# ArturKKK/graphcast-lite

Measured on AMD Instinct MI355X. Metric: training samples/sec (6h windows) + achieved HBM GB/s on mesh GCNConv, higher is better.
Workload: dtype f32

## Files before the change

### graphcast-lite_amd/csrc/linear.hip

```cpp
#include "common.h"
#include "mfma_io.h"
#include "x3.h"

namespace {

using namespace gcl::mfma_io;

#include "gemm_tile.h"

#define gcl_lin_sync() ((abl & 8) != 0)

constexpr int lin_min_waves(int NS, int KT) { return (NS <= 2 && KT <= 64) ? 3 : (NS <= 2 && KT <= 128) ? 2 : 1; }
constexpr bool lin_zpre(int NS, int EPI) { return EPI == 1 && NS >= 4; }

template <int NS, int EPI, int KT, bool VEC>
__global__ __launch_bounds__(256, lin_min_waves(NS, KT)) void linear_mfma_kernel(const float* __restrict__ X, int64_t ldx,
                                                          const float* __restrict__ in_slope,
                                                          const float* __restrict__ W, int32_t ldw, int32_t trans,
                                                          const float* __restrict__ bias, float* __restrict__ Y,
                                                          int64_t ldy, int64_t rows, int32_t K, int32_t N,
                                                          const float* __restrict__ Z, int64_t ldz,
                                                          const float* __restrict__ z_slope,
                                                          double* __restrict__ slope_part, int32_t akind,
                                                          int32_t abl) {
// ... 1032 lines not shown
  g->KT = K <= 64 ? 64 : K <= 128 ? 128 : 256;
  const int KP = ((K + 3) & ~3) + 2;
  g->waves = 4;
  g->lds = ((size_t)g->NS * 32 + 128) * KP * sizeof(float) + 64;
  if (g->lds > gcl::kLdsBytes) {
    g->waves = 2;
    g->lds = ((size_t)g->NS * 32 + 64) * KP * sizeof(float) + 64;
  }
  GCL_CHECK_ARG(g->lds <= gcl::kLdsBytes, "linear: K=%d N=%d needs %zu B of LDS (>160 KiB)", K, N, g->lds);
  int bpc = (int)(gcl::kLdsBytes / g->lds);
  const int by_regs = lin_min_waves(g->NS, g->KT) * 4 / g->waves;
  if (bpc > by_regs) bpc = by_regs;
  if (bpc < 1) bpc = 1;
  const int64_t ntiles = gcl::cdiv(rows, 32 * g->waves);
  const int64_t cap = (int64_t)gcl::kNumCU * bpc;
  g->grid = (int)(ntiles < cap ? ntiles : cap);
  return GCL_OK;
}

template <int EPI>
int launch_linear(const float* X, int64_t ldx, const float* in_slope, const float* W, int ldw, int trans,
                  const float* bias, float* Y, int64_t ldy, int64_t rows, int K, int N, const float* Z, int64_t ldz,
                  const float* z_slope, double* slope_part, int* nparts, hipStream_t st, int akind) {
  if (rows == 0) {
    if (nparts) *nparts = 0;
    return GCL_OK;
  }
  if (use_valu()) {
    const int64_t total = rows * N;
    int grid = (int)(gcl::cdiv(total, 256) < 4096 ? gcl::cdiv(total, 256) : 4096);
    hipLaunchKernelGGL((linear_valu_kernel<EPI>), dim3(grid), dim3(256), 0, st, X, ldx, in_slope, W, ldw, trans,
                       bias, Y, ldy, rows, K, N, Z, ldz, z_slope, slope_part, akind);
    GCL_CHECK_LAUNCH();
    if (nparts) *nparts = grid;
    return GCL_OK;
  }
  const int vec_x = (K % 4 == 0) && (ldx % 4 == 0) && gcl::aligned16(X);
  LinGeom g;
  int rc = lin_geom(rows, K, N, vec_x != 0, &g);
  if (rc) return rc;
#define GCL_LIN3(NS_, KT_, V_)                                                                                    \
  do {                                                                                                            \
    auto kern = linear_mfma_kernel<NS_, EPI, KT_, V_>;                                                            \
    GCL_ENSURE_DYN_LDS(kern, gcl::kLdsBytes);                                                                     \
    hipLaunchKernelGGL(kern, dim3(g.grid), dim3(g.waves * 64), g.lds, st, X, ldx, in_slope, W, ldw, trans, bias,  \
                       Y, ldy, rows, K, N, Z, ldz, z_slope, slope_part, akind, gcl_ablate());                     \
  } while (0)
#define GCL_LIN2(NS_, KT_)                 \
  do {                                     \
    if (vec_x) GCL_LIN3(NS_, KT_, true);   \
    else GCL_LIN3(NS_, KT_, false);        \
  } while (0)
#define GCL_LIN(NS_)                                \
  do {                                              \
    if (g.KT == 64) GCL_LIN2(NS_, 64);              \
    else if (g.KT == 128) GCL_LIN2(NS_, 128);       \
    else GCL_LIN3(NS_, 256, true);                  \
  } while (0)
  switch (g.NS) {
    case 1: GCL_LIN(1); break;
    case 2: GCL_LIN(2); break;
    case 4: GCL_LIN(4); break;
    default: GCL_LIN(8); break;
  }
#undef GCL_LIN3
#undef GCL_LIN
#undef GCL_LIN2
  GCL_CHECK_LAUNCH();
  if (nparts) *nparts = g.grid;
  return GCL_OK;
}

bool panel_fits(int K, int N, bool vec_x, bool trans, bool w_ok) {
  const int impl = gcl::env_is("GCL_DENSE_IMPL", "tile") ? 1 : gcl::env_is("GCL_DENSE_IMPL", "panel") ? 2 : 0;
  const bool tile_ok = vec_x && w_ok && K % 4 == 0 && N % 4 == 0;
  if (impl == 1 && tile_ok) return false;
  if (impl == 0 && tile_ok && (K > 128 || (N >= 128 && (K >= 128 || trans)))) return false;
  if (K < 1 || K > 256 || N < 1 || N > 256) return false;
  if (!vec_x && K > 128) return false;
  int NS = (N + 31) / 32;
  if (NS == 3) NS = 4;
  if (NS > 4) NS = 8;
  const int KP = ((K + 3) & ~3) + 2;
  return ((size_t)NS * 32 + 64) * KP * sizeof(float) + 64 <= gcl::kLdsBytes;
}

template <int EPI>
int launch_gemm(const float* X, int64_t ldx, int akind, const float* slope, const float* W, int64_t ldw, int trans,
                const float* bias, float* Y, int64_t ldy, int64_t rows, int K, int N, const float* Z, int64_t ldz,
                const float* add, int64_t ldadd, double* slope_part, int* nparts, hipStream_t st) {
  if (nparts) *nparts = 0;
  if (rows == 0) return GCL_OK;
  GCL_CHECK_ARG((K % 4 == 0) && (ldx % 4 == 0) && gcl::aligned16(X), "dense: wide shapes need K %% 4 == 0 and 16-B aligned rows (K=%d ldx=%lld)", K, (long long)ldx);
  GCL_CHECK_ARG((ldw % 4 == 0) && gcl::aligned16(W) && (!trans || N % 4 == 0), "dense: wide shapes need a 16-B aligned weight block (ldw=%lld N=%d)", (long long)ldw, N);
  GtGeom g = gt_geom(rows, N);
  const int x3_tile = gcl::env_int("GCL_X3", 1) != 0 && gcl::env_int("GCL_X3_TILE", 1) != 0;
  if (x3_tile && !trans && g.mi == 2) {
    auto kern = gemm_tile_x3_kernel<EPI>;
    GCL_ENSURE_DYN_LDS(kern, gcl::kLdsBytes);
    hipLaunchKernelGGL(kern, dim3(g.grid), dim3(256), gtx3_lds(), st, X, ldx, akind, slope, W, ldw, bias, Y, ldy, rows, K, N,
                       Z, ldz, add, ldadd, slope_part, g.nt, g.total, g.per_xcd);
    GCL_CHECK_LAUNCH();
    if (nparts) *nparts = (int)g.grid;
    return GCL_OK;
  }
#define GCL_GT(T_, MI_)                                                                                           \
  do {                                                                                                            \
    auto kern = gemm_tile_kernel<EPI, T_, MI_>;                                                                   \
    GCL_ENSURE_DYN_LDS(kern, gcl::kLdsBytes);                                                                     \
    hipLaunchKernelGGL(kern, dim3(g.grid), dim3(256), gt_lds(MI_), st, X, ldx, akind, slope, W, ldw, bias, Y, ldy, \
                       rows, K, N, Z, ldz, add, ldadd, slope_part, g.nt, g.total, g.per_xcd);                     \
  } while (0)
  if (trans) {
    if (g.mi == 1) GCL_GT(true, 1);
    else GCL_GT(true, 2);
  } else {
    if (g.mi == 1) GCL_GT(false, 1);
    else GCL_GT(false, 2);
  }
#undef GCL_GT
  GCL_CHECK_LAUNCH();
  if (nparts) *nparts = (int)g.grid;
  return GCL_OK;
}

}

extern "C" size_t gcl_colsum_ws_bytes(int64_t, int32_t);
extern "C" int gcl_colsum(const float*, int64_t, int64_t, int32_t, float*, int32_t, void*, size_t, gcl_stream_t);

static int check_act(const char* who, int act, const float* slope) {
  GCL_CHECK_ARG(act == GCL_ACT_NONE || act == GCL_ACT_PRELU || act == GCL_ACT_SILU, "%s: unknown activation %d", who, act);
  GCL_CHECK_ARG(act != GCL_ACT_PRELU || slope, "%s: GCL_ACT_PRELU needs the slope pointer", who);
  return GCL_OK;
}

extern "C" int gcl_dense_fwd(const float* x, int64_t ldx, int32_t act, const float* slope, const float* W, int64_t ldw,
                             const float* bias, const float* addend, int64_t ldadd, float* y, int64_t ldy,
                             int64_t rows, int32_t Fin, int32_t Fout, gcl_stream_t stream) {
  GCL_CHECK_ARG(x && W && y, "dense_fwd: null argument");
  GCL_CHECK_ARG(rows >= 0 && Fin >= 1 && Fout >= 1 && ldx >= Fin && ldy >= Fout && ldw >= Fin && (!addend || ldadd >= Fout),
                "dense_fwd: bad shape rows=%lld ldx=%lld ldy=%lld ldw=%lld", (long long)rows, (long long)ldx,
                (long long)ldy, (long long)ldw);
  if (int rc = check_act("dense_fwd", act, slope)) return rc;
  const bool vec_x = (Fin % 4 == 0) && (ldx % 4 == 0) && gcl::aligned16(x);
  if (!addend && ldw == Fin && !use_valu() && gcl::x3_linear_fwd_applicable(x, ldx, y, ldy, Fin, Fout, act))
    return gcl::x3_linear_fwd(x, ldx, act, act == GCL_ACT_PRELU ? slope : nullptr, W, bias, y, ldy, rows, Fin, Fout,
                              (hipStream_t)stream);
  if (!addend && ldw == Fin && (use_valu() || panel_fits(Fin, Fout, vec_x, false, (ldw % 4 == 0) && gcl::aligned16(W))))
    return launch_linear<EPI_BIAS>(x, ldx, act == GCL_ACT_PRELU ? slope : nullptr, W, Fin, 0, bias, y, ldy, rows, Fin,
                                   Fout, nullptr, 0, nullptr, nullptr, nullptr, (hipStream_t)stream, act);
  return launch_gemm<EPI_BIAS>(x, ldx, act, act == GCL_ACT_PRELU ? slope : nullptr, W, ldw, 0, bias, y, ldy, rows, Fin,
                               Fout, nullptr, 0, addend, ldadd, nullptr, nullptr, (hipStream_t)stream);
}

extern "C" int gcl_linear_fwd(const float* x, int64_t ldx, const float* in_slope, const float* W, const float* bias,
                              float* y, int64_t ldy, int64_t rows, int32_t Fin, int32_t Fout, gcl_stream_t stream) {
  return gcl_dense_fwd(x, ldx, in_slope ? GCL_ACT_PRELU : GCL_ACT_NONE, in_slope, W, Fin, bias, nullptr, 0, y, ldy, rows,
                       Fin, Fout, stream);
}

static size_t slope_parts_cap(int64_t rows, int32_t Fin) {
  const int64_t g = (int64_t)gt_geom(rows, Fin).grid;
  return (size_t)(g > 4096 ? g : 4096);
}

extern "C" size_t gcl_linear_bwd_ws_bytes(int64_t rows, int32_t Fin, int32_t Fout) {
  size_t nc = (size_t)(Fin + 31) / 32;
  if (nc > 4) nc = 4;
  const size_t FinP = nc * 32;
  size_t no = (size_t)(Fout + 31) / 32;
  no = no <= 2 ? no : no <= 4 ? 4 : 8;
  const size_t FoutP = no * 32;
  const size_t dw = (size_t)kDwBlocks * FoutP * (FinP + 1) * sizeof(float);
  const size_t sl = slope_parts_cap(rows, Fin) * sizeof(double);
  return dw + sl;
}

extern "C" int gcl_dense_bwd_dx(const float* dy, int64_t lddy, const float* W, int64_t ldw, const float* z, int64_t ldz,
                                int32_t act, const float* slope, float* d_slope, const float* addend, int64_t ldadd,
                                float* dx, int64_t lddx, int64_t rows, int32_t Fin, int32_t Fout, void* ws,
                                size_t ws_bytes, gcl_stream_t stream) {
  GCL_CHECK_ARG(dy && W && dx, "dense_bwd_dx: null argument");
  GCL_CHECK_ARG(lddy >= Fout && lddx >= Fin && ldw >= Fin && (!addend || ldadd >= Fin), "dense_bwd_dx: leading dimension too small");
  if (int rc = check_act("dense_bwd_dx", act, slope)) return rc;
  GCL_CHECK_ARG(act == GCL_ACT_NONE || (z && ldz >= Fin), "dense_bwd_dx: activation given without its pre-activation z");
  hipStream_t st = (hipStream_t)stream;
  const float* sl = act == GCL_ACT_PRELU ? slope : nullptr;
  double* slope_part = nullptr;
  if (sl && d_slope) {
    GCL_CHECK_ARG(ws && ws_bytes >= slope_parts_cap(rows, Fin) * sizeof(double) && gcl::aligned16(ws), "dense_bwd_dx: workspace too small");
    slope_part = (double*)ws;
  }
  int nparts = 0, rc;
  const float* zz = act == GCL_ACT_NONE ? nullptr : z;
  const bool vec_x = (Fout % 4 == 0) && (lddy % 4 == 0) && gcl::aligned16(dy);
  if (!addend && ldw == Fin && (use_valu() || panel_fits(Fout, Fin, vec_x, true, (ldw % 4 == 0) && gcl::aligned16(W))))
    rc = launch_linear<EPI_DX>(dy, lddy, nullptr, W, Fin, 1, nullptr, dx, lddx, rows, Fout, Fin, zz, ldz, sl, slope_part,
                               &nparts, st, act);
  else {
    const size_t off = (slope_parts_cap(rows, Fin) * sizeof(double) + 255) & ~(size_t)255;
    const size_t need = off + (size_t)Fin * Fout * sizeof(float);
    if (ws && ws_bytes >= need && gcl::aligned16(ws) && Fout % 4 == 0 && rows >= 4096) {
      float* Wt = reinterpret_cast<float*>(static_cast<char*>(ws) + off);
      hipLaunchKernelGGL(transpose_kernel, dim3((unsigned)gcl::cdiv(Fin, 32), (unsigned)gcl::cdiv(Fout, 32)), dim3(256), 0,
                         st, W, ldw, Wt, Fout, Fin);
      rc = launch_gemm<EPI_DX>(dy, lddy, act, sl, Wt, Fout, 0, nullptr, dx, lddx, rows, Fout, Fin, zz, ldz, addend,
                               ldadd, slope_part, &nparts, st);
    } else {
      rc = launch_gemm<EPI_DX>(dy, lddy, act, sl, W, ldw, 1, nullptr, dx, lddx, rows, Fout, Fin, zz, ldz, addend, ldadd,
                               slope_part, &nparts, st);
    }
  }
  if (rc) return rc;
  if (slope_part && nparts > 0) {
    hipLaunchKernelGGL(reduce_scalar_kernel, dim3(1), dim3(64), 0, st, slope_part, nparts, d_slope);
    GCL_CHECK_LAUNCH();
  }
  return GCL_OK;
}

extern "C" int gcl_linear_bwd_dx(const float* dy, int64_t lddy, const float* W, const float* x, int64_t ldx,
                                 const float* in_slope, float* d_in_slope, float* dx, int64_t lddx, int64_t rows,
                                 int32_t Fin, int32_t Fout, void* ws, size_t ws_bytes, gcl_stream_t stream) {
  GCL_CHECK_ARG(!in_slope || (x && ldx >= Fin), "linear_bwd_dx: in_slope given without the forward input x");
  return gcl_dense_bwd_dx(dy, lddy, W, Fin, in_slope ? x : nullptr, ldx, in_slope ? GCL_ACT_PRELU : GCL_ACT_NONE,
                          in_slope, d_in_slope, nullptr, 0, dx, lddx, rows, Fin, Fout, ws, ws_bytes, stream);
}

static int dw_block(const float* dy, int64_t lddy, const float* x, int64_t ldx, int akind, const float* in_slope,
                    float* dW, int64_t lddw, float* db, int64_t rows, int32_t Fin, int32_t Fout, int32_t accumulate,
                    void* ws, hipStream_t st) {
  const int nct = (Fin + 127) / 128;
  const int NC = nct > 1 ? 4 : (Fin + 31) / 32;
  int NO = (Fout + 31) / 32;
  NO = NO <= 2 ? NO : NO <= 4 ? 4 : 8;
  const int FinP = NC * 32, FoutP = NO * 32;
  const size_t lds = (size_t)kDwRT * (FoutP + FinP) * sizeof(float);
  const int64_t cap = (lds > 80 * 1024 ? gcl::kNumCU : kDwBlocks) / nct;
  int64_t nblk = gcl::cdiv(rows, (nct > 1 ? 4 : 2) * kDwRT);
  if (nblk > cap) nblk = cap;
  if (nblk < 1) nblk = 1;
  int64_t rpb = gcl::cdiv(rows, nblk);
  rpb = gcl::cdiv(rpb, kDwRT) * kDwRT;
  nblk = rows > 0 ? gcl::cdiv(rows, rpb) : 1;
  float* part = (float*)ws;
  float* dbpart = part + (size_t)kDwBlocks * FoutP * FinP;
  const int64_t tile_stride = (int64_t)nblk * FoutP * FinP;
  const bool vec = (lddy % 4 == 0) && (ldx % 4 == 0) && gcl::aligned16(dy) && gcl::aligned16(x);
#define GCL_DW3(NO_, NC_, V_)                                                                                     \
  do {                                                                                                            \
    auto kern = dw_mfma_kernel<NO_, NC_, V_>;                                                                     \
    GCL_ENSURE_DYN_LDS(kern, gcl::kLdsBytes);                                                                     \
    hipLaunchKernelGGL(kern, dim3((unsigned)nblk, (unsigned)nct), dim3(256), lds, st, dy, lddy, x, ldx, in_slope, part, \
                       db ? dbpart : nullptr, rows, Fin, Fout, rpb, akind, tile_stride);                          \
  } while (0)
#define GCL_DW2(NO_, NC_)              \
  do {                                 \
    if (vec) GCL_DW3(NO_, NC_, true);  \
    else GCL_DW3(NO_, NC_, false);     \
  } while (0)
#define GCL_DW(NO_)                    \
  do {                                 \
    switch (NC) {                      \
      case 1: GCL_DW2(NO_, 1); break;  \
      case 2: GCL_DW2(NO_, 2); break;  \
      case 3: GCL_DW2(NO_, 3); break;  \
      default: GCL_DW2(NO_, 4); break; \
    }                                  \
  } while (0)
  switch (NO) {
    case 1: GCL_DW(1); break;
    case 2: GCL_DW(2); break;
    case 4: GCL_DW(4); break;
    default: GCL_DW(8); break;
  }
#undef GCL_DW
#undef GCL_DW2
#undef GCL_DW3
  GCL_CHECK_LAUNCH();
  for (int ct = 0; ct < nct; ct += 3) {
    RedSeg seg[3] = {{nullptr, 0, 0, 1, 0, 0, 0}, {nullptr, 0, 0, 1, 0, 0, 0}, {nullptr, 0, 0, 1, 0, 0, 0}};
    for (int q = 0; q < 3 && ct + q < nct; ++q) {
      const int c = ct + q;
      const int fi = Fin - c * 128 < 128 ? Fin - c * 128 : 128;
      GCL_CHECK_ARG((int64_t)c * tile_stride < ((int64_t)1 << 31), "dense_bwd_dw: partial workspace offset overflows");
      seg[q] = RedSeg{dW + c * 128, (int32_t)(c * tile_stride), Fout * FinP, FinP, fi, (int32_t)lddw, accumulate};
    }
    launch_reduce_multi(part, (int)nblk, (int64_t)FoutP * FinP, seg[0], seg[1], seg[2], st);
    GCL_CHECK_LAUNCH();
  }
  if (db) return gcl::launch_reduce_parts(dbpart, (int)nblk, (int64_t)FoutP, FoutP, db, Fout, 1, Fout, accumulate, st);
  return GCL_OK;
}

extern "C" int gcl_dense_bwd_dw(const float* dy, int64_t lddy, const float* x, int64_t ldx, int32_t act,
                                const float* slope, float* dW, int64_t lddw, float* db, int64_t rows, int32_t Fin,
                                int32_t Fout, int32_t accumulate, void* ws, size_t ws_bytes, gcl_stream_t stream) {
  GCL_CHECK_ARG(dy && x && dW, "dense_bwd_dw: null argument");
  GCL_CHECK_ARG(lddy >= Fout && ldx >= Fin && lddw >= Fin, "dense_bwd_dw: leading dimension too small");
  GCL_CHECK_ARG(Fin >= 1 && Fout >= 1, "dense_bwd_dw: bad shape");
  GCL_CHECK_ARG(lddw < (1 << 30), "dense_bwd_dw: lddw too large");
  if (int rc = check_act("dense_bwd_dw", act, slope)) return rc;
  GCL_CHECK_ARG(ws && ws_bytes >= gcl_linear_bwd_ws_bytes(rows, Fin, Fout), "dense_bwd_dw: workspace too small");
  const float* sl = act == GCL_ACT_PRELU ? slope : nullptr;
  for (int o0 = 0; o0 < Fout; o0 += 256) {
    const int fo = Fout - o0 < 256 ? Fout - o0 : 256;
    int rc = dw_block(dy + o0, lddy, x, ldx, act, sl, dW + (int64_t)o0 * lddw, lddw, db ? db + o0 : nullptr, rows, Fin,
                      fo, accumulate, ws, (hipStream_t)stream);
    if (rc) return rc;
  }
  return GCL_OK;
}

extern "C" int gcl_linear_bwd_dw(const float* dy, int64_t lddy, const float* x, int64_t ldx, const float* in_slope,
                                 float* dW, float* db, int64_t rows, int32_t Fin, int32_t Fout, int32_t accumulate,
                                 void* ws, size_t ws_bytes, gcl_stream_t stream) {
  return gcl_dense_bwd_dw(dy, lddy, x, ldx, in_slope ? GCL_ACT_PRELU : GCL_ACT_NONE, in_slope, dW, Fin, db, rows, Fin,
                          Fout, accumulate, ws, ws_bytes, stream);
}

static bool fused_ok(const float* dy, int64_t lddy, const float* x, int64_t ldx, const float* dx, int64_t lddx,
                     int32_t Fin, int32_t Fout) {
  const int off = gcl::env_int("GCL_NO_FUSED_BWD", 0) != 0;
  if (off || use_valu()) return false;
  return Fout <= 64 && Fin <= 96 && (lddy >= ((Fout + 3) & ~3)) && (Fin % 4 == 0) && (lddy % 4 == 0) && (ldx % 4 == 0) &&
         (lddx >= Fin) && gcl::aligned16(dy) && gcl::aligned16(x) && dx != nullptr;
}

extern "C" size_t gcl_linear_bwd_all_ws_bytes(int64_t rows, int32_t Fin, int32_t Fout) {
  const size_t FiP = (size_t)((Fin + 31) / 32) * 32, FoP = (size_t)((Fout + 31) / 32) * 32;
  const size_t fused = (size_t)3 * gcl::kNumCU * (FoP * FiP + FoP + FiP) * sizeof(float) + (size_t)3 * gcl::kNumCU * 8 + 64;
  size_t sep = gcl_linear_bwd_ws_bytes(rows, Fin, Fout);
  const size_t cs = gcl_colsum_ws_bytes(rows, Fin);
  if (cs > sep) sep = cs;
  return fused > sep ? fused : sep;
}

static int bwd_all_impl(const float* dy, int64_t lddy, const float* W, const float* x, int64_t ldx,
                        const float* in_slope, float* d_in_slope, float* dx, int64_t lddx, float* dW,
                        float* db, float* colsum_dx, int64_t rows, int32_t Fin, int32_t Fout,
                        int32_t accumulate, void* ws, size_t ws_bytes, gcl_stream_t stream, gcl_reduce_job* job) {
  if (job) memset(job, 0, sizeof(*job));
  GCL_CHECK_ARG(dy && W && x && dx && dW, "linear_bwd_all: null argument");
  GCL_CHECK_ARG(ws && ws_bytes >= gcl_linear_bwd_all_ws_bytes(rows, Fin, Fout), "linear_bwd_all: workspace too small");
  hipStream_t st = (hipStream_t)stream;
  const int acc_dw = (accumulate & GCL_ACC_DW) ? 1 : 0, acc_db = (accumulate & GCL_ACC_DB) ? 1 : 0,
            acc_cs = (accumulate & GCL_ACC_COLSUM) ? 1 : 0;
  if (!fused_ok(dy, lddy, x, ldx, dx, lddx, Fin, Fout) || rows == 0) {
    int rc;
    if (db && acc_db != acc_dw) {
      rc = gcl_linear_bwd_dw(dy, lddy, x, ldx, in_slope, dW, nullptr, rows, Fin, Fout, acc_dw, ws, ws_bytes, stream);
      if (rc) return rc;
      rc = gcl_colsum(dy, lddy, rows, Fout, db, acc_db, ws, ws_bytes, stream);
    } else {
      rc = gcl_linear_bwd_dw(dy, lddy, x, ldx, in_slope, dW, db, rows, Fin, Fout, acc_dw, ws, ws_bytes, stream);
    }
    if (rc) return rc;
    rc = gcl_linear_bwd_dx(dy, lddy, W, in_slope ? x : nullptr, ldx, in_slope, d_in_slope, dx, lddx, rows, Fin, Fout,
                           ws, ws_bytes, stream);
    if (rc) return rc;
    if (colsum_dx) rc = gcl_colsum(dx, lddx, rows, Fin, colsum_dx, acc_cs, ws, ws_bytes, stream);
    return rc;
  }
  const int NO = (Fout + 31) / 32, NC = (Fin + 31) / 32;
  const int FoP = NO * 32, FiP = NC * 32;
  const int no64 = gcl::env_int("GCL_NO_FUSED64", 0) != 0;
  const bool use64 = (NC == 2) && !no64;
  const bool use_x3 = use64 && gcl::x3_linear_bwd_applicable(dy, lddy, x, ldx, dx, lddx, Fin, Fout);
  const int64_t ntiles = gcl::cdiv(rows, use64 ? 64 : 128);
  const int64_t cap = use64 ? 3 * gcl::kNumCU : gcl::kNumCU;
  const int nblk = use_x3 ? gcl::x3_linear_bwd_blocks(rows) : (int)(ntiles < cap ? ntiles : cap);
  const size_t rec_f = (size_t)FoP * FiP + FoP + FiP;
  float* part_dw = (float*)ws;
  float* part_db = part_dw + (size_t)FoP * FiP;
  float* part_cs = part_db + FoP;
  double* part_sl = (double*)(((uintptr_t)(part_dw + (size_t)3 * gcl::kNumCU * rec_f) + 15) & ~(uintptr_t)15);
  const bool want_slope = in_slope && d_in_slope;
  if (use_x3) {
    if (int rc = gcl::x3_linear_bwd(dy, lddy, W, x, ldx, in_slope, dx, lddx, rows, Fin, Fout, part_dw, db ? part_db : nullptr,
                                    colsum_dx ? part_cs : nullptr, want_slope ? part_sl : nullptr, st))
      return rc;
  } else if (use64) {
    const size_t lds64 = ((size_t)FiP * (FoP + 2) + 64 * (size_t)(FoP + 2) + 64 * (size_t)FiP) * sizeof(float);
#define GCL_FB64(NO_)                                                                                             \
  do {                                                                                                            \
    auto kern = linear_bwd_fused64_kernel<NO_>;                                                                   \
    hipLaunchKernelGGL(kern, dim3(nblk), dim3(256), lds64, st, dy, lddy, W, x, ldx, in_slope, dx, lddx, rows, Fin, \
                       Fout, part_dw, db ? part_db : nullptr, colsum_dx ? part_cs : nullptr,                      \
                       want_slope ? part_sl : nullptr);                                                           \
  } while (0)
    if (NO == 1) GCL_FB64(1);
    else GCL_FB64(2);
#undef GCL_FB64
  } else {
  const size_t lds = ((size_t)FiP * (FoP + 2) + 128 * (size_t)(FoP + 2) + 128 * (size_t)FiP) * sizeof(float);
#define GCL_FB(NO_, NC_)                                                                                          \
  do {                                                                                                            \
    auto kern = linear_bwd_fused_kernel<NO_, NC_>;                                                                \
    GCL_ENSURE_DYN_LDS(kern, gcl::kLdsBytes);                                                                     \
    hipLaunchKernelGGL(kern, dim3(nblk), dim3(256), lds, st, dy, lddy, W, x, ldx, in_slope, dx, lddx, rows, Fin,  \
                       Fout, part_dw, db ? part_db : nullptr, colsum_dx ? part_cs : nullptr,                      \
                       want_slope ? part_sl : nullptr);                                                           \
  } while (0)
  if (NO == 1 && NC == 1) GCL_FB(1, 1);
  else if (NO == 1 && NC == 2) GCL_FB(1, 2);
  else if (NO == 1 && NC == 3) GCL_FB(1, 3);
  else if (NO == 2 && NC == 1) GCL_FB(2, 1);
  else if (NO == 2 && NC == 2) GCL_FB(2, 2);
  else GCL_FB(2, 3);
#undef GCL_FB
  }
  GCL_CHECK_LAUNCH();
  {
    const int64_t rec = (int64_t)FoP * FiP + FoP + FiP;
    RedSeg s0{dW, 0, Fout * FiP, FiP, Fin, Fin, acc_dw};
    RedSeg s1{db, FoP * FiP, db ? Fout : 0, FoP, Fout, 0, acc_db};
    RedSeg s2{colsum_dx, FoP * FiP + FoP, colsum_dx ? Fin : 0, FiP, Fin, 0, acc_cs};
    if (job) {
      s1.count = db ? FoP : 0;
      s2.count = colsum_dx ? FiP : 0;
      job->part = part_dw;
      job->nparts = nblk;
      job->pstride = rec;
      const RedSeg* ss[3] = {&s0, &s1, &s2};
      for (int q = 0; q < 3; ++q) {
        job->seg[q].out = ss[q]->out;
        job->seg[q].poff = ss[q]->poff;
        job->seg[q].count = ss[q]->count;
        job->seg[q].pld = ss[q]->pld;
        job->seg[q].cols = ss[q]->cols;
        job->seg[q].ldo = ss[q]->ldo;
        job->seg[q].acc = ss[q]->acc;
      }
      job->spart = want_slope ? part_sl : nullptr;
      job->ns = want_slope ? nblk : 0;
      job->sout = want_slope ? d_in_slope : nullptr;
      return GCL_OK;
    }
    launch_reduce_multi(part_dw, nblk, rec, s0, s1, s2, st, want_slope ? part_sl : nullptr, nblk, d_in_slope);
    GCL_CHECK_LAUNCH();
  }
  return GCL_OK;
}

extern "C" int gcl_linear_bwd_all(const float* dy, int64_t lddy, const float* W, const float* x, int64_t ldx,
                                  const float* in_slope, float* d_in_slope, float* dx, int64_t lddx, float* dW,
                                  float* db, float* colsum_dx, int64_t rows, int32_t Fin, int32_t Fout,
                                  int32_t accumulate, void* ws, size_t ws_bytes, gcl_stream_t stream) {
  return bwd_all_impl(dy, lddy, W, x, ldx, in_slope, d_in_slope, dx, lddx, dW, db, colsum_dx, rows, Fin, Fout,
                      accumulate, ws, ws_bytes, stream, nullptr);
}

extern "C" int gcl_linear_bwd_all_deferred(const float* dy, int64_t lddy, const float* W, const float* x, int64_t ldx,
                                           const float* in_slope, float* d_in_slope, float* dx, int64_t lddx,
                                           float* dW, float* db, float* colsum_dx, int64_t rows, int32_t Fin,
                                           int32_t Fout, int32_t accumulate, void* ws, size_t ws_bytes,
                                           gcl_stream_t stream, gcl_reduce_job* job) {
  GCL_CHECK_ARG(job, "linear_bwd_all_deferred: null job");
  return bwd_all_impl(dy, lddy, W, x, ldx, in_slope, d_in_slope, dx, lddx, dW, db, colsum_dx, rows, Fin, Fout,
                      accumulate, ws, ws_bytes, stream, job);
}

extern "C" int gcl_reduce_jobs(const gcl_reduce_job* jobs, int32_t n, gcl_stream_t stream) {
  GCL_CHECK_ARG(n >= 0 && (jobs || n == 0), "reduce_jobs: null argument");
  hipStream_t st = (hipStream_t)stream;
  for (int32_t q = 0; q < n;) {
    RedJobsK J;
    memset(&J, 0, sizeof(J));
    int nb = 0, cnt = 0;
    bool any_slope = false;
    for (; q < n && cnt < kJobsPerLaunch; ++q) {
      const gcl_reduce_job& g = jobs[q];
      if (g.nparts <= 0) continue;
      GCL_CHECK_ARG(g.part && g.pstride % 4 == 0 && gcl::aligned16(g.part), "reduce_jobs: bad partial buffer");
      RedJobK& k = J.j[cnt];
      k.part = g.part;
      k.pstride = g.pstride;
      RedSeg* ss[3] = {&k.s0, &k.s1, &k.s2};
      int total = 0;
      for (int t = 0; t < 3; ++t) {
        GCL_CHECK_ARG((g.seg[t].poff | g.seg[t].count) % 4 == 0, "reduce_jobs: segment not 16-byte granular");
        *ss[t] = RedSeg{g.seg[t].out, g.seg[t].poff, g.seg[t].out ? g.seg[t].count : 0, g.seg[t].pld > 0 ? g.seg[t].pld : 1,
                        g.seg[t].cols, g.seg[t].ldo, g.seg[t].acc};
        total += ss[t]->count;
      }
      k.spart = g.spart;
      k.sout = g.sout;
      k.nparts = g.nparts;
      k.ns = g.ns;
      k.blk0 = nb;
      any_slope = any_slope || (g.spart && g.sout && g.ns > 0);
      if (!(g.spart && g.sout && g.ns > 0)) k.spart = nullptr;
      nb += (int)gcl::cdiv(total, 32);
      ++cnt;
    }
    if (cnt == 0) continue;
    J.n = cnt;
    J.nblk = nb;
    hipLaunchKernelGGL(reduce_jobs_kernel, dim3((unsigned)nb + (any_slope ? 1u : 0u)), dim3(256), 0, st, J);
    GCL_CHECK_LAUNCH();
  }
  return GCL_OK;
}
```

### graphcast-lite_amd/csrc/linear_x3.hip

```cpp
#include "mfma_io.h"
#include "x3.h"

namespace {

typedef unsigned int u32x2 __attribute__((ext_vector_type(2)));

#ifndef GCL_X3_ST_AUX
#define GCL_X3_ST_AUX 2
#endif
__device__ __forceinline__ float4 ld_stream(const float4* p) {
#ifndef GCL_X3_LD_PLAIN
  typedef float lv4f __attribute__((ext_vector_type(4)));
  const lv4f v = __builtin_nontemporal_load(reinterpret_cast<const lv4f*>(p));
  return make_float4(v.x, v.y, v.z, v.w);
#else
  return *p;
#endif
}
using namespace gcl::mfma_io;
using namespace gcl::x3;

constexpr int kRowB = 144;
constexpr int kImgB = 32 * kRowB;
constexpr int kTileB = 3 * kImgB;

__device__ unsigned long long x3_stamps[8 * 4096];
#ifdef GCL_STAMPS
#define X3_STAMP(slot)                                                           \
  do {                                                                           \
    __builtin_amdgcn_sched_barrier(0);                                           \
    unsigned long long t_;                                                       \
    asm volatile("s_memtime %0\n\ts_waitcnt lgkmcnt(0)" : "=s"(t_)::"memory"); \
    __builtin_amdgcn_sched_barrier(0);                                           \
    stamp_acc[slot] += t_ - stamp_last;                                          \
    stamp_last = t_;                                                             \
  } while (0)
#else
#define X3_STAMP(slot) do {} while (0)
#endif

template <int NS, bool SILU, int NKS>
__global__ __launch_bounds__(256, 2) void linear_x3_fwd_kernel(const float* __restrict__ X, int64_t ldx,
                                                               const float* __restrict__ slope_p, int32_t akind,
                                                               const float* __restrict__ W,
                                                               const float* __restrict__ bias, float* __restrict__ Y,
                                                               int64_t ldy, int64_t rows, int32_t K, int32_t N,
                                                               int32_t abl) {
  extern __shared__ __align__(16) unsigned char smem8[];
#ifdef GCL_STAMPS
  const unsigned long long stamp_t0 = __builtin_amdgcn_s_memtime();
#endif
  const int tid = threadIdx.x, lane = tid & 63, wave = __builtin_amdgcn_readfirstlane(tid >> 6);
  unsigned char* Aw = smem8 + wave * kTileB;
  const int fo = (lane & 31) * kRowB + (lane >> 5) * 16;
  const bool no_mfma = (abl & 2) != 0;
  const int64_t rows_ld = (abl & 4) ? 0 : rows;

  bf16x8 wf[NS][NKS][3];
  {
    constexpr int kWimgB = NS * 32 * kRowB;
    float2 wv[NS * 4];
#pragma unroll
    for (int i = 0; i < NS * 4; ++i) {
      const int idx = i * 256 + tid;
      const int j = idx >> 5, k = (idx & 31) * 2;
      const bool okj = j < N;
      wv[i].x = (okj && k < K) ? W[(int64_t)j * K + k] : 0.f;
      wv[i].y = (okj && k + 1 < K) ? W[(int64_t)j * K + k + 1] : 0.f;
    }
#pragma unroll
    for (int i = 0; i < NS * 4; ++i) {
      const int idx = i * 256 + tid;
      const int j = idx >> 5, k = (idx & 31) * 2;
      const Pk3 p = split2(wv[i].x, wv[i].y);
      unsigned char* d = smem8 + j * kRowB + k * 2;
      *reinterpret_cast<unsigned*>(d) = p.h;
      *reinterpret_cast<unsigned*>(d + kWimgB) = p.m;
      *reinterpret_cast<unsigned*>(d + 2 * kWimgB) = p.l;
    }
    __syncthreads();
#pragma unroll
    for (int t = 0; t < NS; ++t)
#pragma unroll
      for (int s = 0; s < NKS; ++s)
#pragma unroll
        for (int p = 0; p < 3; ++p)
          wf[t][s][p] = *reinterpret_cast<const bf16x8*>(smem8 + p * kWimgB + t * 32 * kRowB + fo + s * 32);
    __syncthreads();
  }

  const float pa = (akind == gcl::kActPrelu) ? *slope_p : 1.f;
  float4 bq;
  {
    const int oc = (lane % (NS * 8)) * 4;
    bq.x = (bias && oc < N) ? bias[oc] : 0.f;
    bq.y = (bias && oc + 1 < N) ? bias[oc + 1] : 0.f;
    bq.z = (bias && oc + 2 < N) ? bias[oc + 2] : 0.f;
    bq.w = (bias && oc + 3 < N) ? bias[oc + 3] : 0.f;
  }

  const int rsub = lane >> 4, csub = lane & 15;
  const bool cok = csub * 4 < K;
  float4 pre[8];
  auto issue = [&](int64_t tile) {
    const int64_t r0 = tile * 128 + wave * 32;
#pragma unroll
    for (int it = 0; it < 8; ++it) {
      const int64_t row = r0 + it * 4 + rsub;
      const float4* p = (cok && row < rows_ld) ? reinterpret_cast<const float4*>(X + row * ldx + csub * 4) : zero4;
      pre[it] = ld_stream(p);
    }
  };
  auto commit = [&]() {
#pragma unroll
    for (int it = 0; it < 8; ++it) {
      float4 v = pre[it];
      if (SILU) {
        v.x = gcl::silu_f(v.x); v.y = gcl::silu_f(v.y); v.z = gcl::silu_f(v.z); v.w = gcl::silu_f(v.w);
      } else {
        const float mx = v.x * pa, my = v.y * pa, mz = v.z * pa, mw = v.w * pa;
        v.x = v.x > 0.f ? v.x : mx; v.y = v.y > 0.f ? v.y : my;
        v.z = v.z > 0.f ? v.z : mz; v.w = v.w > 0.f ? v.w : mw;
      }
      const Pk3 p01 = split2(v.x, v.y), p23 = split2(v.z, v.w);
      unsigned char* d = Aw + (it * 4 + rsub) * kRowB + csub * 8;
      *reinterpret_cast<u32x2*>(d) = u32x2{p01.h, p23.h};
      *reinterpret_cast<u32x2*>(d + kImgB) = u32x2{p01.m, p23.m};
      *reinterpret_cast<u32x2*>(d + 2 * kImgB) = u32x2{p01.l, p23.l};
    }
  };

  const int64_t ntiles = (rows + 127) / 128;
  issue(blockIdx.x);
#ifdef GCL_STAMPS
  unsigned long long stamp_acc[8] = {0, 0, 0, 0, 0, 0, 0, 0}, stamp_last = __builtin_amdgcn_s_memtime();
  stamp_acc[6] = stamp_last - stamp_t0;
  stamp_acc[7] = stamp_t0;
#endif
  for (int64_t t = blockIdx.x; t < ntiles; t += gridDim.x) {
    __builtin_amdgcn_fence(__ATOMIC_ACQ_REL, "wavefront");
    X3_STAMP(0);
#ifdef GCL_STAMPS
    asm volatile("s_waitcnt vmcnt(0)" ::: "memory");
#endif
    X3_STAMP(1);
    commit();
    X3_STAMP(2);
    issue(t + gridDim.x);
    X3_STAMP(3);

    f32x16 acc[NS];
#pragma unroll
    for (int s = 0; s < NS; ++s)
#pragma unroll
      for (int r = 0; r < 16; ++r) acc[s][r] = 0.f;
    if (!no_mfma) {
#pragma unroll
      for (int s = 0; s < NKS; ++s) {
        const unsigned char* ap = Aw + fo + s * 32;
        const bf16x8 ah = *reinterpret_cast<const bf16x8*>(ap);
        const bf16x8 am = *reinterpret_cast<const bf16x8*>(ap + kImgB);
        const bf16x8 al = *reinterpret_cast<const bf16x8*>(ap + 2 * kImgB);
#pragma unroll
        for (int c = 0; c < NS; ++c) acc[c] = mfma_lo(acc[c], ah, am, al, wf[c][s][0], wf[c][s][1], wf[c][s][2]);
      }
#pragma unroll
      for (int s = 0; s < NKS; ++s) {
        const unsigned char* ap = Aw + fo + s * 32;
        const bf16x8 ah = *reinterpret_cast<const bf16x8*>(ap);
        const bf16x8 am = *reinterpret_cast<const bf16x8*>(ap + kImgB);
#pragma unroll
        for (int c = 0; c < NS; ++c) acc[c] = mfma_mid(acc[c], ah, am, wf[c][s][0], wf[c][s][1]);
      }
#pragma unroll
      for (int s = 0; s < NKS; ++s) {
        const bf16x8 ah = *reinterpret_cast<const bf16x8*>(Aw + fo + s * 32);
#pragma unroll
        for (int c = 0; c < NS; ++c) acc[c] = mfma_hi(acc[c], ah, wf[c][s][0]);
      }
    }

#ifdef GCL_STAMPS
    asm volatile("" ::"v"(acc[0][0]));
#endif
    X3_STAMP(4);
    const int64_t r0 = t * 128 + wave * 32;
    const int64_t nr64 = rows - r0;
    const int nr = nr64 < 0 ? 0 : (nr64 < 32 ? (int)nr64 : 32);
    constexpr int OS = NS * 32, LPO = OS / 4, RPP = 64 / LPO;
    float* Ot = reinterpret_cast<float*>(Aw);
#pragma unroll
    for (int s = 0; s < NS; ++s)
#pragma unroll
      for (int r = 0; r < 16; ++r) Ot[d_row(r, lane) * OS + s * 32 + (lane & 31)] = acc[s][r];
    const __amdgpu_buffer_rsrc_t ry = make_rsrc(Y + r0 * ldy, (nr > 0 && !(abl & 1)) ? ((int64_t)(nr - 1) * ldy + N) * 4 : 0);
    const int orow = lane / LPO, ocol = (lane % LPO) * 4;
#pragma unroll
    for (int p = 0; p < 32 / RPP; ++p) {
      const int i = p * RPP + orow;
      float4 v = *reinterpret_cast<const float4*>(Ot + i * OS + ocol);
      v.x += bq.x; v.y += bq.y; v.z += bq.z; v.w += bq.w;
      buf_st4<GCL_X3_ST_AUX>(ry, (ocol < N) ? (unsigned)((i * ldy + ocol) * 4) : kOOB, v);
    }
    X3_STAMP(5);
  }
#ifdef GCL_STAMPS
  if (lane == 0 && blockIdx.x < 1024)
    for (int i = 0; i < 8; ++i) x3_stamps[(blockIdx.x * 4 + wave) * 8 + i] = stamp_acc[i];
#endif
}

constexpr int kBRowB = 128;
constexpr int kImg64B = 64 * kBRowB;
__device__ __forceinline__ int swz(int r) { return (((r >> 1) & 1) << 2) | (((r >> 3) & 1) << 1) | ((r >> 2) & 1); }
__device__ __forceinline__ int sw_off(int r, int b) { return r * kBRowB + ((((b >> 4) ^ swz(r)) << 4) | (b & 15)); }

typedef short s16x4 __attribute__((ext_vector_type(4)));
__device__ __forceinline__ bf16x8 tr_frag(const unsigned char* base, int o0, int o1) {
  typedef __attribute__((address_space(3))) s16x4 lds_s16x4;
  const s16x4 a = __builtin_amdgcn_ds_read_tr16_b64_v4i16((lds_s16x4*)(base + o0));
  const s16x4 b = __builtin_amdgcn_ds_read_tr16_b64_v4i16((lds_s16x4*)(base + o1));
  return __builtin_shufflevector(a, b, 0, 1, 2, 3, 4, 5, 6, 7);
}

template <int NO>
__global__ __launch_bounds__(256, 2) void linear_x3_bwd_kernel(
    const float* __restrict__ dY, int64_t lddy, const float* __restrict__ W, const float* __restrict__ P,
    int64_t ldp, const float* __restrict__ in_slope, float* __restrict__ dX, int64_t lddx, int64_t rows, int32_t Fin,
    int32_t Fout, float* __restrict__ part_dw, float* __restrict__ part_db, float* __restrict__ part_cs,
    double* __restrict__ part_slope) {
  constexpr int FoP = NO * 32, FiP = 64, NKO = NO * 2, NT = NO * 2;
  extern __shared__ __align__(16) unsigned char smem8[];
  unsigned char* Yimg = smem8;
  unsigned char* Pimg = smem8 + 3 * kImg64B;
  float* Stg = reinterpret_cast<float*>(smem8 + 6 * kImg64B);
  const int tid = threadIdx.x, lane = tid & 63, wave = __builtin_amdgcn_readfirstlane(tid >> 6);
  const int li = lane & 31, h = lane >> 5;
  const int rg = wave & 1, sg = wave >> 1;
  const int so = wave % NO, sc = wave / NO;
  const bool has_tile = wave < NT;

  bf16x8 wtf[NKO][3];
  {
    float2 wv[8];
#pragma unroll
    for (int i = 0; i < 8; ++i) {
      const int idx = i * 256 + tid;
      const int c = idx & 63, o = (idx >> 6) * 2;
      wv[i].x = (c < Fin && o < Fout) ? W[(int64_t)o * Fin + c] : 0.f;
      wv[i].y = (c < Fin && o + 1 < Fout) ? W[(int64_t)(o + 1) * Fin + c] : 0.f;
    }
#pragma unroll
    for (int i = 0; i < 8; ++i) {
      const int idx = i * 256 + tid;
      const int c = idx & 63, o = (idx >> 6) * 2;
      const Pk3 p = split2(wv[i].x, wv[i].y);
      unsigned char* d = Yimg + sw_off(c, o * 2);
      *reinterpret_cast<unsigned*>(d) = p.h;
      *reinterpret_cast<unsigned*>(d + kImg64B) = p.m;
      *reinterpret_cast<unsigned*>(d + 2 * kImg64B) = p.l;
    }
    __syncthreads();
#pragma unroll
    for (int s = 0; s < NKO; ++s)
#pragma unroll
      for (int p = 0; p < 3; ++p)
        wtf[s][p] = *reinterpret_cast<const bf16x8*>(Yimg + p * kImg64B + sw_off(32 * sg + li, (16 * s + 8 * h) * 2));
    __syncthreads();
  }

  const bool act = in_slope != nullptr;
  const float slope = act ? *in_slope : 1.f;
  const int64_t ntiles = (rows + 63) / 64;

  const int rsub = lane >> 4, csub = lane & 15;
  const bool yok = csub * 4 < Fout, pok = csub * 4 < Fin;
  const unsigned ym0 = csub * 4 < Fout ? ~0u : 0u, ym1 = csub * 4 + 1 < Fout ? ~0u : 0u, ym2 = csub * 4 + 2 < Fout ? ~0u : 0u,
                 ym3 = csub * 4 + 3 < Fout ? ~0u : 0u;
  float4 pre_y[4], pre_p[4];
  auto issue = [&](int64_t tile) {
    const int64_t r0 = tile * 64 + wave * 16;
#pragma unroll
    for (int it = 0; it < 4; ++it) {
      const int64_t row = r0 + it * 4 + rsub;
      const bool rok = row < rows;
      pre_y[it] = ld_stream((yok && rok) ? reinterpret_cast<const float4*>(dY + row * lddy + csub * 4) : zero4);
      pre_p[it] = ld_stream((pok && rok) ? reinterpret_cast<const float4*>(P + row * ldp + csub * 4) : zero4);
    }
  };

  int fo[NKO];
#pragma unroll
  for (int s = 0; s < NKO; ++s) fo[s] = sw_off(rg * 32 + li, (2 * s + h) * 16);
  const int g = lane >> 4, i16 = lane & 15;
  int troY[2], troP[2];
#pragma unroll
  for (int j = 0; j < 2; ++j) {
    const int r = 8 * (g >> 1) + 4 * j + (i16 >> 2), b = 32 * (g & 1) + 8 * (i16 & 3);
    troY[j] = sw_off(r, 64 * so + b);
    troP[j] = sw_off(r, 64 * sc + b);
  }

  f32x16 dw_hi, dw_lo;
#pragma unroll
  for (int r = 0; r < 16; ++r) dw_hi[r] = 0.f, dw_lo[r] = 0.f;
  float4 db4 = make_float4(0.f, 0.f, 0.f, 0.f), cs4 = make_float4(0.f, 0.f, 0.f, 0.f);
  double slope_acc = 0.0;
  float4 cur_p[4];

  issue(blockIdx.x);
#ifdef GCL_STAMPS
  unsigned long long stamp_acc[8] = {0, 0, 0, 0, 0, 0, 0, 0}, stamp_last = __builtin_amdgcn_s_memtime();
#endif
  for (int64_t t = blockIdx.x; t < ntiles; t += gridDim.x) {
#ifdef GCL_STAMPS
    asm volatile("s_waitcnt vmcnt(0)" ::: "memory");
#endif
    X3_STAMP(0);
#pragma unroll
    for (int it = 0; it < 4; ++it) {
      float4 y = pre_y[it];
      y.x = __uint_as_float(__float_as_uint(y.x) & ym0); y.y = __uint_as_float(__float_as_uint(y.y) & ym1);
      y.z = __uint_as_float(__float_as_uint(y.z) & ym2); y.w = __uint_as_float(__float_as_uint(y.w) & ym3);
      db4.x += y.x; db4.y += y.y; db4.z += y.z; db4.w += y.w;
      const float4 z = pre_p[it];
      cur_p[it] = z;
      float4 a;
      {
        const float mx = z.x * slope, my = z.y * slope, mz = z.z * slope, mw = z.w * slope;
        a.x = z.x > 0.f ? z.x : mx; a.y = z.y > 0.f ? z.y : my; a.z = z.z > 0.f ? z.z : mz; a.w = z.w > 0.f ? z.w : mw;
      }
      const Pk3 y01 = split2(y.x, y.y), y23 = split2(y.z, y.w), a01 = split2(a.x, a.y), a23 = split2(a.z, a.w);
      const int off = sw_off(wave * 16 + it * 4 + rsub, csub * 8);
      *reinterpret_cast<u32x2*>(Yimg + off) = u32x2{y01.h, y23.h};
      *reinterpret_cast<u32x2*>(Yimg + off + kImg64B) = u32x2{y01.m, y23.m};
      *reinterpret_cast<u32x2*>(Yimg + off + 2 * kImg64B) = u32x2{y01.l, y23.l};
      *reinterpret_cast<u32x2*>(Pimg + off) = u32x2{a01.h, a23.h};
      *reinterpret_cast<u32x2*>(Pimg + off + kImg64B) = u32x2{a01.m, a23.m};
      *reinterpret_cast<u32x2*>(Pimg + off + 2 * kImg64B) = u32x2{a01.l, a23.l};
    }
    X3_STAMP(1);
    __syncthreads();
    X3_STAMP(2);
    issue(t + gridDim.x);
    X3_STAMP(3);

    {
      f32x16 acc;
#pragma unroll
      for (int r = 0; r < 16; ++r) acc[r] = 0.f;
#pragma unroll
      for (int s = 0; s < NKO; ++s) {
        const bf16x8 ah = *reinterpret_cast<const bf16x8*>(Yimg + fo[s]);
        const bf16x8 am = *reinterpret_cast<const bf16x8*>(Yimg + fo[s] + kImg64B);
        const bf16x8 al = *reinterpret_cast<const bf16x8*>(Yimg + fo[s] + 2 * kImg64B);
        acc = mfma_lo(acc, ah, am, al, wtf[s][0], wtf[s][1], wtf[s][2]);
      }
#pragma unroll
      for (int s = 0; s < NKO; ++s) {
        const bf16x8 ah = *reinterpret_cast<const bf16x8*>(Yimg + fo[s]);
        const bf16x8 am = *reinterpret_cast<const bf16x8*>(Yimg + fo[s] + kImg64B);
        acc = mfma_mid(acc, ah, am, wtf[s][0], wtf[s][1]);
      }
#pragma unroll
      for (int s = 0; s < NKO; ++s) acc = mfma_hi(acc, *reinterpret_cast<const bf16x8*>(Yimg + fo[s]), wtf[s][0]);
#pragma unroll
      for (int r = 0; r < 16; ++r) Stg[(rg * 32 + d_row(r, lane)) * 64 + sg * 32 + li] = acc[r];
    }

    X3_STAMP(4);
    if (has_tile) {
#pragma unroll
      for (int s = 0; s < 4; ++s) {
        const unsigned char* ya = Yimg + s * 16 * kBRowB;
        const unsigned char* pa = Pimg + s * 16 * kBRowB;
        const bf16x8 ah = tr_frag(ya, troY[0], troY[1]), am = tr_frag(ya + kImg64B, troY[0], troY[1]),
                     al = tr_frag(ya + 2 * kImg64B, troY[0], troY[1]);
        const bf16x8 bh = tr_frag(pa, troP[0], troP[1]), bm = tr_frag(pa + kImg64B, troP[0], troP[1]),
                     bl = tr_frag(pa + 2 * kImg64B, troP[0], troP[1]);
        dw_lo = mfma_lo(dw_lo, ah, am, al, bh, bm, bl);
        dw_lo = mfma_mid(dw_lo, ah, am, bh, bm);
        dw_hi = mfma_hi(dw_hi, ah, bh);
      }
    }
#ifdef GCL_STAMPS
    asm volatile("" ::"v"(dw_hi[0]), "v"(dw_lo[0]));
#endif
    X3_STAMP(5);
    __syncthreads();
    X3_STAMP(6);

    {
      const int64_t r0 = t * 64;
      const int64_t nr = (rows - r0) < 64 ? (rows - r0) : 64;
      const __amdgpu_buffer_rsrc_t rx = make_rsrc(dX + r0 * lddx, nr > 0 ? ((nr - 1) * lddx + Fin) * 4 : 0);
#pragma unroll
      for (int it = 0; it < 4; ++it) {
        const int row = wave * 16 + it * 4 + rsub;
        float4 v = *reinterpret_cast<const float4*>(Stg + row * 64 + csub * 4);
        const float4 z = cur_p[it];
        const bool nx = act && z.x <= 0.f, ny = act && z.y <= 0.f, nz = act && z.z <= 0.f, nw = act && z.w <= 0.f;
        slope_acc += (double)(((nx ? v.x * z.x : 0.f) + (ny ? v.y * z.y : 0.f)) + ((nz ? v.z * z.z : 0.f) + (nw ? v.w * z.w : 0.f)));
        v.x = nx ? v.x * slope : v.x; v.y = ny ? v.y * slope : v.y; v.z = nz ? v.z * slope : v.z; v.w = nw ? v.w * slope : v.w;
        cs4.x += v.x; cs4.y += v.y; cs4.z += v.z; cs4.w += v.w;
        buf_st4<GCL_X3_ST_AUX>(rx, pok ? (unsigned)((row * lddx + csub * 4) * 4) : kOOB, v);
      }
    }
    X3_STAMP(7);
  }
#ifdef GCL_STAMPS
  if (lane == 0 && blockIdx.x < 1024)
    for (int i = 0; i < 8; ++i) x3_stamps[(blockIdx.x * 4 + wave) * 8 + i] = stamp_acc[i];
#endif

  constexpr size_t REC = (size_t)FoP * FiP + FoP + FiP;
  float* out = part_dw + (size_t)blockIdx.x * REC;
  if (has_tile) {
#pragma unroll
    for (int r = 0; r < 16; ++r) out[(size_t)(so * 32 + d_row(r, lane)) * FiP + sc * 32 + li] = dw_hi[r] + dw_lo[r];
  }
  __syncthreads();
  float* red = reinterpret_cast<float*>(smem8);
  {
    float* rdb = red + (wave * 4 + rsub) * 64 + csub * 4;
    *reinterpret_cast<float4*>(rdb) = db4;
    *reinterpret_cast<float4*>(rdb + 16 * 64) = cs4;
  }
  for (int off = 32; off > 0; off >>= 1) slope_acc += __shfl_down(slope_acc, off, 64);
  double* dred = reinterpret_cast<double*>(red + 2 * 16 * 64);
  if (lane == 0) dred[wave] = slope_acc;
  __syncthreads();
  if (tid < 128) {
    const int which = tid >> 6, c = tid & 63;
    float s = 0.f;
#pragma unroll
    for (int q = 0; q < 16; ++q) s += red[(which * 16 + q) * 64 + c];
    if (which == 0) {
      if (part_db && c < FoP) part_db[(size_t)blockIdx.x * REC + c] = s;
    } else {
      if (part_cs) part_cs[(size_t)blockIdx.x * REC + c] = s;
    }
  }
  if (part_slope && tid == 0) part_slope[blockIdx.x] = (dred[0] + dred[1]) + (dred[2] + dred[3]);
}

int x3_ablate() {
#ifndef GCL_STAMPS
  return 0;
#endif
  static const int v = gcl::env_int("GCL_ABLATE", 0);
  return v;
}

}

#ifdef GCL_STAMPS
extern "C" int gcl_debug_read_stamps_x3(unsigned long long* host_out, int count) {
  GCL_CHECK_HIP(hipDeviceSynchronize());
  GCL_CHECK_HIP(hipMemcpyFromSymbol(host_out, HIP_SYMBOL(x3_stamps), sizeof(unsigned long long) * count));
  return GCL_OK;
}
#endif

namespace gcl {

bool x3_linear_fwd_applicable(const float* x, int64_t ldx, const float* y, int64_t ldy, int K, int N, int akind) {
  if (!env_int("GCL_X3", 1)) return false;
  if (K < 1 || K > 64 || N < 4 || N > 64 || (N & 3)) return false;
  if ((ldx & 3) || (ldy & 3) || !aligned16(x) || !aligned16(y)) return false;
  if (ldx * 4 * 35 >= ((int64_t)1 << 31) || ldy * 4 * 35 >= ((int64_t)1 << 31)) return false;
  return akind == kActNone || akind == kActPrelu || akind == kActSilu;
}

int x3_linear_fwd(const float* x, int64_t ldx, int akind, const float* slope, const float* W, const float* bias,
                  float* y, int64_t ldy, int64_t rows, int K, int N, hipStream_t st) {
  if (rows == 0) return GCL_OK;
  const int64_t ntiles = cdiv(rows, 128);
  const int grid = (int)(ntiles < 2 * kNumCU ? ntiles : 2 * kNumCU);
  const size_t lds = 4 * (size_t)kTileB;
#define GCL_X3F3(NS_, SILU_, NKS_)                                                                                \
  hipLaunchKernelGGL((linear_x3_fwd_kernel<NS_, SILU_, NKS_>), dim3(grid), dim3(256), lds, st, x, ldx, slope, akind, \
                     W, bias, y, ldy, rows, K, N, x3_ablate())
#define GCL_X3F(NS_, SILU_)           \
  do {                                \
    if (K <= 32) GCL_X3F3(NS_, SILU_, 2); \
    else GCL_X3F3(NS_, SILU_, 4);     \
  } while (0)
  if (akind == kActSilu) {
    if (N > 32) GCL_X3F(2, true);
    else GCL_X3F(1, true);
  } else {
    if (N > 32) GCL_X3F(2, false);
    else GCL_X3F(1, false);
  }
#undef GCL_X3F3
#undef GCL_X3F
  GCL_CHECK_LAUNCH();
  return GCL_OK;
}

bool x3_linear_bwd_applicable(const float* dy, int64_t lddy, const float* x, int64_t ldx, const float* dx, int64_t lddx,
                              int Fin, int Fout) {
  if (!env_int("GCL_X3", 1)) return false;
  if (Fin < 33 || Fin > 64 || (Fin & 3) || Fout < 1 || Fout > 64) return false;
  if (lddy < ((Fout + 3) & ~3) || (lddy & 3) || (ldx & 3) || (lddx & 3) || lddx < Fin) return false;
  if (!aligned16(dy) || !aligned16(x) || !aligned16(dx)) return false;
  return lddx * 4 * 70 < ((int64_t)1 << 31);
}

int x3_linear_bwd_blocks(int64_t rows) {
  const int64_t ntiles = cdiv(rows, 64);
  return (int)(ntiles < 2 * kNumCU ? ntiles : 2 * kNumCU);
}

int x3_linear_bwd(const float* dy, int64_t lddy, const float* W, const float* x, int64_t ldx, const float* in_slope,
                  float* dx, int64_t lddx, int64_t rows, int Fin, int Fout, float* part_dw, float* part_db,
                  float* part_cs, double* part_slope, hipStream_t st) {
  const int grid = x3_linear_bwd_blocks(rows);
  const size_t lds = 6 * (size_t)kImg64B + 64 * 64 * sizeof(float);
#define GCL_X3B(NO_)                                                                                              \
  do {                                                                                                            \
    auto kern = linear_x3_bwd_kernel<NO_>;                                                                        \
    GCL_ENSURE_DYN_LDS(kern, gcl::kLdsBytes);                                                                     \
    hipLaunchKernelGGL(kern, dim3(grid), dim3(256), lds, st, dy, lddy, W, x, ldx, in_slope, dx, lddx, rows, Fin, Fout, \
                       part_dw, part_db, part_cs, part_slope);                                                    \
  } while (0)
  if (Fout > 32) GCL_X3B(2);
  else GCL_X3B(1);
#undef GCL_X3B
  GCL_CHECK_LAUNCH();
  return GCL_OK;
}

}
```

### graphcast-lite_amd/csrc/x3.h

```cpp
#pragma once
#include "common.h"

namespace gcl {

bool x3_linear_fwd_applicable(const float* x, int64_t ldx, const float* y, int64_t ldy, int K, int N, int akind);
int x3_linear_fwd(const float* x, int64_t ldx, int akind, const float* slope, const float* W, const float* bias,
                  float* y, int64_t ldy, int64_t rows, int K, int N, hipStream_t st);

bool x3_linear_bwd_applicable(const float* dy, int64_t lddy, const float* x, int64_t ldx, const float* dx, int64_t lddx,
                              int Fin, int Fout);
int x3_linear_bwd_blocks(int64_t rows);
int x3_linear_bwd(const float* dy, int64_t lddy, const float* W, const float* x, int64_t ldx, const float* in_slope,
                  float* dx, int64_t lddx, int64_t rows, int Fin, int Fout, float* part_dw, float* part_db,
                  float* part_cs, double* part_slope, hipStream_t st);

}

#ifdef __HIPCC__
#include "mfma_io.h"

namespace gcl {
namespace x3 {

using mfma_io::f32x16;
typedef short bf16x8 __attribute__((ext_vector_type(8)));
typedef __bf16 bf16x2_t __attribute__((ext_vector_type(2)));
typedef float f32x2_t __attribute__((ext_vector_type(2)));

__device__ __forceinline__ unsigned pk_bf16(float a, float b) {
  return __builtin_bit_cast(unsigned, __builtin_convertvector(f32x2_t{a, b}, bf16x2_t));
}
struct Pk3 {
  unsigned h, m, l;
};
__device__ __forceinline__ Pk3 split2(float a, float b) {
  Pk3 p;
  p.h = pk_bf16(a, b);
  float ra = a - __uint_as_float(p.h << 16), rb = b - __uint_as_float(p.h & 0xffff0000u);
  p.m = pk_bf16(ra, rb);
  ra -= __uint_as_float(p.m << 16);
  rb -= __uint_as_float(p.m & 0xffff0000u);
  p.l = pk_bf16(ra, rb);
  return p;
}

__device__ __forceinline__ f32x16 mfma_lo(f32x16 acc, bf16x8 ah, bf16x8 am, bf16x8 al, bf16x8 bh, bf16x8 bm, bf16x8 bl) {
  acc = __builtin_amdgcn_mfma_f32_32x32x16_bf16(al, bh, acc, 0, 0, 0);
  acc = __builtin_amdgcn_mfma_f32_32x32x16_bf16(ah, bl, acc, 0, 0, 0);
  acc = __builtin_amdgcn_mfma_f32_32x32x16_bf16(am, bm, acc, 0, 0, 0);
  return acc;
}
__device__ __forceinline__ f32x16 mfma_mid(f32x16 acc, bf16x8 ah, bf16x8 am, bf16x8 bh, bf16x8 bm) {
  acc = __builtin_amdgcn_mfma_f32_32x32x16_bf16(am, bh, acc, 0, 0, 0);
  acc = __builtin_amdgcn_mfma_f32_32x32x16_bf16(ah, bm, acc, 0, 0, 0);
  return acc;
}
__device__ __forceinline__ f32x16 mfma_hi(f32x16 acc, bf16x8 ah, bf16x8 bh) {
  return __builtin_amdgcn_mfma_f32_32x32x16_bf16(ah, bh, acc, 0, 0, 0);
}

}
}
#endif
```

### graphcast-lite_amd/functional.py

```python
from typing import List, Optional

import os

import torch

from . import hip


def _grad_slot(p: Optional[torch.Tensor], needs: bool):
    if p is None or not needs:
        return None, False, True
    if p.grad is not None:
        return p.grad, True, True
    return torch.zeros_like(p), False, False


class _Grads:

    def __init__(self, params: List[Optional[torch.Tensor]], needs: List[bool]):
        self.dst, self.acc, self.ret_none = [], [], []
        for p, nd in zip(params, needs):
            d, a, r = _grad_slot(p, nd)
            self.dst.append(d)
            self.acc.append(a)
            self.ret_none.append(r)

    def out(self):
        return tuple(None if r else d for d, r in zip(self.dst, self.ret_none))


def _flat3(x: torch.Tensor):
    if x.dim() == 2:
        x = x.unsqueeze(0)
    if not x.is_contiguous():
        x = x.contiguous()
    return x


class MLPFn(torch.autograd.Function):
    @staticmethod
    def forward(ctx, x, owner, has_ln: bool, eps: float, *params):
        L = (len(params) - (2 if has_ln else 0) + 1) // 3
        shape = x.shape
        x2 = hip.rows2d(x.detach())
        zs = []
        cur, slope = x2, None
        for k in range(L):
            W, b = params[3 * k], params[3 * k + 1]
            z = hip.linear_fwd(cur, W.detach(), b.detach(), slope)
            zs.append(z)
            cur = z
            slope = params[3 * k + 2].detach() if k < L - 1 else None
        stats = None
        out = cur
        if has_ln:
            out, stats = hip.layernorm_fwd(cur, params[-2].detach(), params[-1].detach(), eps)
        ctx.owner, ctx.has_ln, ctx.L = owner, has_ln, L
        ctx.x2, ctx.zs, ctx.stats = x2, zs, stats
        ctx.params = params
        return out.view(shape[:-1] + (out.shape[-1],))

    @staticmethod
    def backward(ctx, dy):
        params, L = ctx.params, ctx.L
        needs = list(ctx.needs_input_grad[4:])
        G = _Grads(list(params), needs)
        dy2 = hip.rows2d(dy)
        zs = ctx.zs
        if ctx.has_ln:
            gi, bi = len(params) - 2, len(params) - 1
            dgam = G.dst[gi] if G.dst[gi] is not None else torch.zeros_like(params[gi])
            dbet = G.dst[bi] if G.dst[bi] is not None else torch.zeros_like(params[bi])
            dz = hip.layernorm_bwd(dy2, zs[-1], params[gi].detach(), ctx.stats, dgam, dbet, G.acc[gi] and G.acc[bi])
        else:
            dz = dy2
        dx = None
        for k in range(L - 1, -1, -1):
            W = params[3 * k].detach()
            inp = ctx.x2 if k == 0 else zs[k - 1]
            slope = None if k == 0 else params[3 * k - 1].detach()
            wi, bi = 3 * k, 3 * k + 1
            dW = G.dst[wi] if G.dst[wi] is not None else torch.zeros_like(params[wi])
            db = G.dst[bi]
            if k > 0:
                dz = hip.linear_bwd_all(dz, W, inp, slope, G.dst[3 * k - 1], dW, db, None, G.acc[wi], acc_db=G.acc[bi])
            elif ctx.needs_input_grad[0]:
                dx = hip.linear_bwd_all(dz, W, inp, None, None, dW, db, None, G.acc[wi], acc_db=G.acc[bi],
                                        act=hip.ACT_NONE)
            elif db is not None and G.acc[bi] != G.acc[wi]:
                hip.linear_bwd_dw(dz, inp, None, dW, None, G.acc[wi])
                hip.colsum(dz, db, G.acc[bi])
            else:
                hip.linear_bwd_dw(dz, inp, None, dW, db, G.acc[wi])
        if dx is not None:
            dx = dx.view(dy.shape[:-1] + (dx.shape[-1],))
        return (dx, None, None, None) + G.out()


_LN_COLSUM = os.environ.get("GCL_NO_LN_COLSUM", "0") in ("0", "")
_ROWS_OUT = os.environ.get("GCL_NO_ROWS_OUT", "0") in ("0", "")


def _lat_first_layer_bwd(lat, enc3, dz3, W, dW, acc_dw: bool, want_dx: bool, Pc=None, enc_shape=None):
    _, _, inv_a, inv_fold = lat.maps
    B, ne, D = enc_shape if enc3 is None else enc3.shape
    G, Md, r = lat.G, lat.Md, lat.r
    nc = Md + r
    Fo = dz3.shape[-1]
    dz3 = dz3 if dz3.is_contiguous() else dz3.contiguous()
    dzc = torch.empty(B, nc, Fo, dtype=torch.float32, device=dz3.device)
    if Md > 0:
        hip.gather2_rows(dz3, inv_a[G: G + Md], None, None, Md, B, out=dzc[:, :Md])
    if r > 1:
        hip.gather2_rows(dz3, inv_fold, None, None, B * r, B, sum_batch=True, out=dzc[:, Md:], deal=r)
    elif r == 1:
        tmp = hip.gather2_rows(dz3, inv_fold, None, None, B * r, B, sum_batch=True)
        hip.copy_rows(tmp.view(B, r, Fo), dzc[:, Md:])
    if Pc is None:
        Pc = hip.copy_rows(enc3[:, G:, :], torch.empty(B, nc, D, dtype=torch.float32, device=dz3.device))
    land = lat.landing
    shared = land is not None and land.buf is not None
    if not want_dx:
        hip.linear_bwd_dw(dzc.view(B * nc, Fo), Pc.view(B * nc, D), None, dW, None, acc_dw)
        dxc = None
    else:
        dxc = hip.linear_bwd_all(dzc.view(B * nc, Fo), W, Pc.view(B * nc, D), None, None, dW, None, None, acc_dw,
                                 act=hip.ACT_NONE).view(B, nc, D)
    if shared:
        if dxc is not None:
            hip.copy_rows(dxc, land.buf[:, G:])
        land.buf, land.mesh_pending, land.handed_over = None, False, False
        return None
    if dxc is None:
        return None
    out = torch.zeros(B, ne, D, dtype=torch.float32, device=dz3.device)
    hip.copy_rows(dxc, out[:, G:])
    return out


class LatSource:

    def __init__(self, tab, maps, M: int, G: int, Md: int, r: int, landing=None):
        self.tab, self.maps, self.M, self.G, self.Md, self.r, self.landing = tab, maps, M, G, Md, r, landing
        self._compact = {}

    def compact_tab(self, ne: int):
        t = self._compact.get(ne)
        if t is None:
            tab = self.tab.to(torch.int64)
            f = -tab - 1
            bq = torch.div(f, ne, rounding_mode="floor")
            flat_c = bq * (self.Md + self.r) + (f - bq * ne - self.G)
            t = torch.where(tab >= 0, tab - self.G, -flat_c - 1).to(torch.int32).contiguous()
            self._compact[ne] = t
        return t


class GCNStackFn(torch.autograd.Function):
    @staticmethod
    def forward(ctx, x, owner, graph, L: int, has_ln: bool, eps: float, out_rows: int, *params):
        squeeze = x.dim() == 2
        x3 = _flat3(x.detach())
        B, n, _ = x3.shape
        lat = getattr(owner, "_lat_src", None)
        if lat is not None:
            owner._lat_src = None
            n = lat.M
            if not x3.is_contiguous():
                x3 = x3.contiguous()
            if lat.landing is not None:
                lat.landing.mesh_pending = True
        ctx.lat = lat
        slope_p = params[2 * L]
        akind = getattr(owner, "act_kind", hip.ACT_PRELU)
        slope_t = slope_p.detach() if slope_p is not None else getattr(owner, "const_slope", None)
        ps = []
        cur = x3
        pad_last = None
        for k in range(L):
            W, b = params[2 * k].detach(), params[2 * k + 1].detach()
            Fout = W.shape[0]
            ldh = (Fout + 3) // 4 * 4
            act_k, slope_k = (akind, slope_t) if k > 0 else (hip.ACT_NONE, None)
            if k == 0 and lat is not None:
                p = hip.gcn_layer_fwd_tab(graph, x3, lat.tab, act_k, slope_k, W, b)
                if ldh != Fout:
                    p = p.contiguous()
                ps.append(p)
                cur = p
                continue
            if hip.gcn_layer_fusable(graph, cur, W.shape[1], Fout):
                last_rows = int(out_rows) if (k == L - 1 and out_rows and out_rows < n and not has_ln and _ROWS_OUT) else None
                p = hip.gcn_layer_fwd(graph, cur, act_k, slope_k, W, b, rows_out=last_rows)
                if k == L - 1 and ldh != Fout and not has_ln:
                    pad_last = (ldh, Fout, None)
                elif ldh != Fout:
                    p = p.contiguous()
                ps.append(p)
                cur = p
                continue
            if k == L - 1 and ldh != Fout and not has_ln:
                Wp = torch.nn.functional.pad(W, (0, 0, 0, ldh - Fout))
                bp = torch.nn.functional.pad(b, (0, ldh - Fout))
                h = hip.linear_fwd(cur.reshape(B * n, -1), Wp, None, slope_k, act=act_k)
                p = hip.aggregate(graph, h.view(B, n, ldh), bp)
                ps.append(p)
                cur = p[..., :Fout]
                pad_last = (ldh, Fout, Wp)
                continue
            h = hip.linear_fwd(cur.reshape(B * n, -1) if not cur.is_contiguous() else cur.view(B * n, -1), W, None, slope_k,
                               ld_out=ldh, act=act_k)
            h3 = torch.as_strided(h, (B, n, Fout), (n * ldh, ldh, 1))
            p = hip.aggregate(graph, h3, b)
            ps.append(p)
            cur = p
        ctx.akind, ctx.slope_t, ctx.pad_last = akind, slope_t, pad_last
        out, stats = cur, None
        ctx.land = getattr(owner, "_grad_src", None)
        if ctx.land is not None:
            owner._grad_src = None
            if has_ln and not (out_rows and out_rows < n) and not squeeze:
                ctx.land.proc_ready = True
            else:
                ctx.land = None
        if has_ln:
            land = ctx.land
            if land is not None and land.dec_buf is not None and cur.is_contiguous() and land.dec_buf.shape[2] == cur.shape[2]:
                stats = hip.layernorm_fwd_map(cur.view(B * n, -1), params[-2].detach(), params[-1].detach(), eps,
                                              land.dec_buf, land.dec_map)
                land.dec_filled = True
                out = cur.new_zeros(()).expand(B, n, cur.shape[2])
            else:
                o2, stats = hip.layernorm_fwd(cur.view(B * n, -1), params[-2].detach(), params[-1].detach(), eps)
                out = o2.view(B, n, -1)
        ctx.owner, ctx.graph, ctx.L, ctx.has_ln = owner, graph, L, has_ln
        ctx.x3, ctx.ps, ctx.stats, ctx.params, ctx.squeeze = x3, ps, stats, params, squeeze
        ctx.n_rows, ctx.out_rows = n, (int(out_rows) if out_rows and out_rows < n else 0)
        if ctx.out_rows:
            out = out[:, :ctx.out_rows, :]
        return out[0] if squeeze else out

    @staticmethod
    def backward(ctx, dy):
        params, L, graph = ctx.params, ctx.L, ctx.graph
        needs = list(ctx.needs_input_grad[7:])
        G = _Grads(list(params), needs)
        land = ctx.land
        dy_map = None
        if land is not None and land.proc_src is not None:
            if all(st == 0 for st in dy.stride()):
                dy_map = (land.proc_src, land.proc_map)
                dy3 = dy
            else:
                src, pmap = land.proc_src, land.proc_map
                dy3 = _flat3(dy) + hip.gather2_rows(src, pmap, None, None, dy.shape[-2], src.shape[0])
            land.proc_src = land.proc_map = None
            land.proc_ready = False
        else:
            dy3 = _flat3(dy)
        B, n = dy3.shape[0], ctx.n_rows
        ps = ctx.ps
        pad = ctx.pad_last
        dy_rows = dy3
        if ctx.out_rows and (ctx.has_ln or pad is None):
            dy3 = hip.pad_rows(dy3, n, dy3.shape[2])
        bi_last = 2 * L - 1
        cs_done = False
        if ctx.has_ln:
            gi, bi = len(params) - 2, len(params) - 1
            dgam = G.dst[gi] if G.dst[gi] is not None else torch.zeros_like(params[gi])
            dbet = G.dst[bi] if G.dst[bi] is not None else torch.zeros_like(params[bi])
            cs = G.dst[bi_last] if (pad is None and _LN_COLSUM) else None
            dp = hip.layernorm_bwd(None if dy_map is not None else dy3.view(B * n, -1), ps[-1].view(B * n, -1),
                                   params[gi].detach(), ctx.stats, dgam, dbet, G.acc[gi] and G.acc[bi], colsum_dx=cs,
                                   acc_colsum=bool(cs is not None and G.acc[bi_last]), dy_map=dy_map).view(B, n, -1)
            cs_done = cs is not None
        else:
            dp = dy3
        si = 2 * L
        dsl = G.dst[si] if params[si] is not None else None
        slope_t, akind = ctx.slope_t, ctx.akind
        dx = None
        Fo = params[2 * (L - 1)].shape[0]
        Fp = Fo
        if pad is not None:
            Fp = pad[0]
            dp = hip.pad_rows(dy_rows if not ctx.has_ln else dp, n, Fp)
        if G.dst[bi_last] is not None and not cs_done:
            src = dy_rows if not ctx.has_ln else dp[..., :Fo]
            hip.colsum(src.reshape(-1, Fo), G.dst[bi_last], G.acc[bi_last])
        for k in range(L - 1, -1, -1):
            W = params[2 * k].detach()
            wi = 2 * k
            inp = (ctx.x3 if k == 0 else ps[k - 1]).view(-1, (ctx.x3 if k == 0 else ps[k - 1]).shape[-1])
            dh2 = hip.aggregate(graph, dp, None, transpose=True).view(B * n, -1)
            if k == L - 1 and Fp != Fo:
# ... 470 lines not shown
```

### graphcast-lite_amd/hip.py

```python
import ctypes as C
import os
from typing import Optional

import torch

_HERE = os.path.dirname(os.path.abspath(__file__))
LIB_PATH = os.environ.get("GCL_LIB") or os.path.join(_HERE, "libgcl_hip.so")

GRAPH_GCN, GRAPH_GAT, GRAPH_MEAN = 0, 1, 2

_lib = None

_i32, _i64, _f32, _vp, _sz = C.c_int32, C.c_int64, C.c_float, C.c_void_p, C.c_size_t

_SIGNATURES = {
    "gcl_version": (C.c_int, []),
    "gcl_last_error": (C.c_char_p, []),
    "gcl_graph_count_edges": (C.c_int, [_vp, _i64, _i32, _i32, C.POINTER(_i64)]),
    "gcl_graph_build_host": (C.c_int, [_vp, _i64, _i32, _i32] + [_vp] * 8),
    "gcl_graph_create": (C.c_int, [_vp, _i64, _i32, _i32, C.POINTER(_vp)]),
    "gcl_graph_destroy": (None, [_vp]),
    "gcl_graph_num_nodes": (_i32, [_vp]),
    "gcl_graph_num_edges": (_i64, [_vp]),
    "gcl_graph_max_in_degree": (_i32, [_vp]),
    "gcl_graph_export_edges": (C.c_int, [_vp, _vp]),
    "gcl_graph_eperm_device": (_vp, [_vp]),
    "gcl_graph_halo_info": (C.c_int, [_vp, _i32, _i32, _vp]),
    "gcl_linear_fwd": (C.c_int, [_vp, _i64, _vp, _vp, _vp, _vp, _i64, _i64, _i32, _i32, _vp]),
    "gcl_linear_bwd_dx": (C.c_int, [_vp, _i64, _vp, _vp, _i64, _vp, _vp, _vp, _i64, _i64, _i32, _i32, _vp, _sz, _vp]),
    "gcl_linear_bwd_dw": (C.c_int, [_vp, _i64, _vp, _i64, _vp, _vp, _vp, _i64, _i32, _i32, _i32, _vp, _sz, _vp]),
    "gcl_linear_bwd_ws_bytes": (_sz, [_i64, _i32, _i32]),
    "gcl_linear_bwd_all": (C.c_int, [_vp, _i64, _vp, _vp, _i64, _vp, _vp, _vp, _i64, _vp, _vp, _vp, _i64, _i32, _i32,
                                     _i32, _vp, _sz, _vp]),
    "gcl_linear_bwd_all_deferred": (C.c_int, [_vp, _i64, _vp, _vp, _i64, _vp, _vp, _vp, _i64, _vp, _vp, _vp, _i64, _i32,
                                              _i32, _i32, _vp, _sz, _vp, _vp]),
    "gcl_reduce_jobs": (C.c_int, [_vp, _i32, _vp]),
    "gcl_linear_bwd_all_ws_bytes": (_sz, [_i64, _i32, _i32]),
    "gcl_aggregate": (C.c_int, [_vp, _i32, _vp, _i64, _i64, _vp, _vp, _i64, _i64, _i32, _i32, _vp]),
    "gcl_gat_fwd": (C.c_int, [_vp, _vp, _i64, _i64, _vp, _vp, _vp, _vp, _vp, _vp, _vp, _i64, _i64, _i32, _i32, _i32, _vp]),
    "gcl_gat_bwd": (C.c_int, [_vp, _vp, _i64, _i64, _vp, _i64, _i64, _vp, _vp, _vp, _vp, _vp, _vp, _i64, _i64,
                              _vp, _vp, _vp, _i32, _i32, _i32, _i32, _vp, _sz, _vp]),
    "gcl_gat_bwd_ws_bytes": (_sz, [_i64, _i32, _i32, _i32, _i32]),
    "gcl_gat_fwd_tab": (C.c_int, [_vp, _vp, _i64, _i64, _vp, _vp, _vp, _vp, _vp, _vp, _vp, _vp, _i64, _i64, _i32, _i32, _i32, _vp]),
    "gcl_gat_bwd_tab": (C.c_int, [_vp, _vp, _i64, _i64, _vp, _i64, _i64, _vp, _vp, _vp, _vp, _vp, _vp, _vp, _i64, _i64,
                                  _vp, _vp, _vp, _i32, _i32, _i32, _i32, _vp, _sz, _vp]),
    "gcl_gat_tab_ok": (C.c_int, [_vp, _i64, _i32, _i32]),
    "gcl_gat_alpha_to_edge_order": (C.c_int, [_vp, _vp, _vp, _i32, _vp]),
    "gcl_gat_prune": (C.c_int, [_vp, _vp, _f32, _vp, C.POINTER(_i64), _vp, _sz, _vp]),
    "gcl_gat_prune_ws_bytes": (_sz, [_i64]),
    "gcl_layernorm_fwd": (C.c_int, [_vp, _i64, _vp, _vp, _f32, _vp, _i64, _vp, _i64, _i32, _vp]),
    "gcl_layernorm_bwd": (C.c_int, [_vp, _i64, _vp, _i64, _vp, _vp, _vp, _i64, _vp, _vp, _i32, _i64, _i32, _vp, _sz, _vp]),
    "gcl_layernorm_bwd_cs": (C.c_int, [_vp, _i64, _vp, _i64, _vp, _vp, _vp, _i64, _vp, _vp, _vp, _i32, _i64, _i32, _vp, _sz, _vp]),
    "gcl_layernorm_bwd_map": (C.c_int, [_vp, _i64, _i64, _vp, _i32, _vp, _i64, _vp, _vp, _vp, _i64, _vp, _vp, _vp, _i32, _i64,
                                        _i32, _vp, _sz, _vp]),
    "gcl_layernorm_bwd_ws_bytes": (_sz, [_i64, _i32]),
    "gcl_graphnorm_fwd": (C.c_int, [_vp, _i64, _i64, _vp, _vp, _f32, _vp, _i64, _i64, _vp, _i32, _i32, _i32, _vp, _sz, _vp]),
    "gcl_graphnorm_bwd": (C.c_int, [_vp, _i64, _i64, _vp, _i64, _i64, _vp, _vp, _f32, _vp, _i64, _i64, _vp, _vp,
                                    _i32, _i32, _i32, _i32, _vp, _sz, _vp]),
    "gcl_graphnorm_ws_bytes": (_sz, [_i32, _i32, _i32]),
    "gcl_colsum": (C.c_int, [_vp, _i64, _i64, _i32, _vp, _i32, _vp, _sz, _vp]),
    "gcl_colsum_ws_bytes": (_sz, [_i64, _i32]),
    "gcl_assemble_input": (C.c_int, [_vp, _vp, _vp, _vp, _i64, _i32, _i32, _i32, _i32, _i32, _vp]),
    "gcl_assemble_input_tail": (C.c_int, [_vp, _vp, _vp, _vp, _i32, _vp, _i64, _i32, _i32, _i32, _i32, _i32, _vp]),
    "gcl_wmse_fwd_bwd": (C.c_int, [_vp, _i64, _i64, _vp, _i64, _i64, _vp, _i64, _i64, _vp, _vp, _f32, _f32, _vp,
                                   _vp, _vp, _vp, _i32, _i32, _i32, _vp, _sz, _vp]),
    "gcl_ar_step_bwd": (C.c_int, [_vp, _vp, _vp, _vp, _i32, _i32, _vp, _vp, _i32, _i32, _i32, _i32, _vp]),
    "gcl_pad_rows": (C.c_int, [_vp, _i64, _i64, _i32, _i32, _vp, _i64, _i64, _i32, _i32, _i32, _vp]),
    "gcl_zero": (C.c_int, [_vp, _sz, _vp]),
    "gcl_wmse_ws_bytes": (_sz, [_i32, _i32, _i32]),
    "gcl_adam_step": (C.c_int, [_vp, _vp, _vp, _vp, _i64, _f32, _f32, _f32, _f32, _f32, _i32, _f32, _vp]),
    "gcl_adam_step_dev": (C.c_int, [_vp, _vp, _vp, _vp, _i64, _f32, _f32, _f32, _f32, _f32, _vp, _vp, _f32, _vp]),
    "gcl_adam_step_groups": (C.c_int, [_vp, _vp, _vp, _vp, _i64, _vp, _i32, _vp, _vp, _vp, _vp, _f32, _f32, _f32, _f32,
                                       _f32, _vp]),
    "gcl_copy_rows": (C.c_int, [_vp, _i64, _i64, _vp, _i64, _i64, _i32, _i32, _i32, _vp]),
    "gcl_dense_fwd": (C.c_int, [_vp, _i64, _i32, _vp, _vp, _i64, _vp, _vp, _i64, _vp, _i64, _i64, _i32, _i32, _vp]),
    "gcl_dense_bwd_dx": (C.c_int, [_vp, _i64, _vp, _i64, _vp, _i64, _i32, _vp, _vp, _vp, _i64, _vp, _i64, _i64, _i32, _i32,
                                   _vp, C.c_size_t, _vp]),
    "gcl_dense_bwd_dw": (C.c_int, [_vp, _i64, _vp, _i64, _i32, _vp, _vp, _i64, _vp, _i64, _i32, _i32, _i32, _vp,
                                   C.c_size_t, _vp]),
    "gcl_gcn_layer_fwd": (C.c_int, [_vp, _vp, _i64, _i64, _i32, _vp, _vp, _vp, _vp, _i64, _i64, _i32, _i32, _i32, _i32, _vp]),
    "gcl_gcn_layer_fwd_rows": (C.c_int, [_vp, _vp, _i64, _i64, _i32, _vp, _vp, _vp, _vp, _i64, _i64, _i32, _i32, _i32, _i32, _i32, _vp]),
    "gcl_layernorm_fwd_map": (C.c_int, [_vp, _i64, _vp, _vp, _f32, _vp, _i64, _i64, _vp, _i32, _vp, _i64, _i32, _vp]),
    "gcl_gcn_layer_fwd_tab": (C.c_int, [_vp, _vp, _i64, _i64, _i64, _vp, _i32, _vp, _vp, _vp, _vp, _i64, _i64, _i32, _i32, _i32, _i32, _vp]),
    "gcl_gcn_layer_fwd_tab_ok": (C.c_int, [_vp, _i64, _i64, _i64, _i32, _i32, _i32]),
    "gcl_segment_reduce": (C.c_int, [_vp, _i64, _i64, _vp, _vp, _i32, _vp, _i64, _i64, _i32, _i32, _i32, _vp]),
    "gcl_edge_combine": (C.c_int, [_vp, _vp, _vp, _i64, _i64, _vp, _vp, _vp, _i64, _i64, _vp, _vp, _i32, _i64, _i32, _vp]),
    "gcl_act_fwd": (C.c_int, [_vp, _vp, _i64, _i32, _vp, _vp]),
    "gcl_act_bwd": (C.c_int, [_vp, _vp, _vp, _i64, _i32, _vp, _vp, _vp, C.c_size_t, _vp]),
    "gcl_act_bwd_ws_bytes": (C.c_size_t, []),
    "gcl_window_pack": (C.c_int, [_vp, _i64, _i32, _i32, _i32, _vp, _vp, _vp, _i32, _i32, _i32, _vp, _vp, _i32, _vp]),
    "gcl_ar_advance": (C.c_int, [_vp, _vp, _i64, _i64, _vp, _i64, _i64, _vp, _vp, _vp, _i64, _i64, _i32, _i32, _i32, _i32,
                                 _i32, _i32, _vp]),
    "gcl_gather2_rows": (C.c_int, [_vp, _i64, _i64, _vp, _vp, _i64, _i64, _vp, _vp, _i64, _i64, _i32, _i32, _i32, _i32, _vp]),
    "gcl_roi_gather_rows": (C.c_int, [_vp, _i32, _i32] + [_vp, _i64, _i64, _i32] * 3 + [_vp, _i64, _i64, _i32, _i32, _vp]),
    "gcl_roi_compose": (C.c_int, [_vp, _i64, _i64, _vp, _i64, _i64, _vp, _vp, _i64, _i64, _i32, _i32, _i32, _vp]),
    "gcl_segment_wsum": (C.c_int, [_vp, _i64, _i64, _i32, _i32, _vp, _vp, _vp, _vp, _i64, _i64, _vp, _i64, _i64, _i32,
                                   _i32, _i32, _i32, _vp]),
    "gcl_cross_update_fwd": (C.c_int, [_vp, _i64, _i64, _vp, _i64, _i64, _vp, _vp, _vp, _f32, _vp, _vp, _vp, _i32, _i32,
                                       _i32, _vp]),
    "gcl_nudge": (C.c_int, [_vp, _i64, _i64, _vp, _i64, _i64, _vp, _f32, _f32, _i32, _vp, _i64, _i64, _i32, _i32, _i32,
                            _vp]),
    "gcl_oi_max_stations": (C.c_int, []),
    "gcl_oi_station_cov": (C.c_int, [_vp, _vp, _i32, C.c_double, C.c_double, C.c_double, _vp, _vp]),
    "gcl_oi_factor": (C.c_int, [_vp, _i32, _vp]),
    "gcl_oi_solve": (C.c_int, [_vp, _i32, _vp, _vp, _vp, _i32, _vp]),
    "gcl_oi_innovation": (C.c_int, [_vp, _i64, _i64, _vp, _i64, _i64, _vp, _vp, _vp, _i32, _i32, _i32, _vp, _vp]),
    "gcl_oi_analysis": (C.c_int, [_vp, _i64, _i64, _vp, _i64, _i64, _vp, _i32, _vp, _vp, _vp, _vp, _i32, _vp, _vp, _vp,
                                  _vp, _i32, _f32, _f32, _f32, _f32, _i32, _vp]),
    "gcl_verify_colstats_ws_bytes": (_sz, [_i32, _i32, _i32, _i32]),
    "gcl_verify_colstats": (C.c_int, [_vp, _i64, _i64, _i32, _i32] + [_vp, _i64, _i64, _vp] * 4
                            + [_vp, _i32, _i32, _vp, _vp, _sz, _vp]),
    "gcl_verify_accumulate": (C.c_int, [_vp, _vp, _i32, _vp, _vp, _vp]),
    "gcl_regrid_blend": (C.c_int, [_vp, _i32, _i64, _i64, _i32, _vp, _vp, _i32, _i32, _vp, _i64, _i64, _vp, _vp, _i64,
                                   _i64, _vp, _i64, _i64, _i32, _vp]),
    "gcl_taper_blend": (C.c_int, [_vp, _vp, _i64, _i64, _vp, _i64, _i64, _vp, _i64, _i64, _i32, _i32, _i32, _vp]),
    "gcl_mos_forest_eval": (C.c_int, [_vp, _vp, _i32, C.c_double, _vp, _i32, _vp, _vp]),
    "gcl_mos_forest_predict": (C.c_int, [_vp, _vp, _i32, C.c_double, _vp, _i32, _i64, _i64, _i64, _i32] + [_i32] * 5
                               + [_vp, _vp, _i32, _i32, _vp, _vp, _vp, _vp, _i32, _vp]),
    "gcl_mos_idw_apply": (C.c_int, [_vp, _i32, _i64, _i64, _i64, _vp, _i64, _i64, _i64, _i32, _i32, _i32, _i32, _vp,
                                    _vp, _vp, _i32, _vp, _i32, C.c_double, C.c_double, _vp, _i32, _vp]),
    "gcl_mos_table_apply": (C.c_int, [_vp, _i32, _i64, _i64, _i64, _vp, _i64, _i64, _i64, _i32, _i32, _i32, _i32, _vp,
                                      _i32, _i32, _vp]),
}


def exported_symbols():
    return sorted(_SIGNATURES)


def lib():
    global _lib
    if _lib is None:
        if not os.path.exists(LIB_PATH):
            raise RuntimeError(
                f"{LIB_PATH} is missing: build it with `python -c 'import __graft_entry__ as g; g.build()'` "
                "(or `make -C graphcast-lite_amd/csrc`). The HIP path has no CPU fallback."
            )
        L = C.CDLL(LIB_PATH)
        for name, (res, args) in _SIGNATURES.items():
            fn = getattr(L, name)
            fn.restype = res
            fn.argtypes = args
        _lib = L
    return _lib


def _check(rc: int):
    if rc != 0:
        raise RuntimeError(f"libgcl_hip error {rc}: {lib().gcl_last_error().decode()}")


def _stream() -> int:
    return torch.cuda.current_stream().cuda_stream


def _p(t: Optional[torch.Tensor]):
    if t is None:
        return None
    if not t.is_cuda:
        raise RuntimeError("libgcl_hip needs GPU tensors (there is no CPU fallback)")
    if t.dtype != torch.float32:
        raise RuntimeError(f"libgcl_hip needs float32 tensors, got {t.dtype}")
    return t.data_ptr()


_ws = {}
_ws_retired = []


def workspace(nbytes: int, device) -> torch.Tensor:
    key = torch.device(device).index if torch.device(device).index is not None else torch.cuda.current_device()
    cur = _ws.get(key)
    if cur is None or cur.numel() < nbytes:
        size = max(int(nbytes), 1 << 20, 2 * cur.numel() if cur is not None else 0)
        if cur is not None:
            _ws_retired.append(cur)
        cur = torch.empty(size, dtype=torch.uint8, device=f"cuda:{key}")
        _ws[key] = cur
    return cur


def rows2d(t: torch.Tensor) -> torch.Tensor:
    if t.dim() == 2 and t.stride(1) == 1:
        return t
    if not t.is_contiguous():
        t = t.contiguous()
    return t.view(-1, t.shape[-1])


# ... 107 lines not shown

def _probe_begin(kind, **info):
    return PROBE.begin(kind, **info) if PROBE is not None else None


def _probe_end(tok):
    if tok is not None:
        PROBE.end(tok)


def dense_fwd(x, W, bias, act=ACT_NONE, slope=None, addend=None, out=None):
    rows, Fin = x.shape
    Fout = W.shape[0]
    assert W.shape[1] == Fin and W.stride(1) == 1 and x.stride(1) == 1
    if out is None:
        out = torch.empty(rows, Fout, dtype=torch.float32, device=x.device)
    if rows == 0:
        return out
    tok = _probe_begin("dense_fwd", rows=rows, Fin=Fin, Fout=Fout)
    _check(lib().gcl_dense_fwd(_p(x), _ld(x), int(act), _p(slope), _p(W), W.stride(0), _p(bias), _p(addend),
                               _ld(addend) if addend is not None else 0, _p(out), _ld(out), rows, Fin, Fout, _stream()))
    _probe_end(tok)
    return out


def dense_bwd_dx(dy, W, z=None, act=ACT_NONE, slope=None, d_slope=None, addend=None, out=None):
    rows, Fout = dy.shape
    Fin = W.shape[1]
    assert W.shape[0] == Fout and W.stride(1) == 1
    if out is None:
        out = torch.empty(rows, Fin, dtype=torch.float32, device=dy.device)
    if rows == 0:
        return out
    nb = lib().gcl_linear_bwd_ws_bytes(rows, Fin, Fout)
    ws = workspace(nb, dy.device)
    _check(lib().gcl_dense_bwd_dx(_p(dy), _ld(dy), _p(W), W.stride(0), _p(z), _ld(z) if z is not None else 0, int(act),
                                  _p(slope), _p(d_slope), _p(addend), _ld(addend) if addend is not None else 0, _p(out),
                                  _ld(out), rows, Fin, Fout, ws.data_ptr(), ws.numel(), _stream()))
    return out


def dense_bwd_dw(dy, x, dW, db, accumulate: bool, act=ACT_NONE, slope=None):
    rows, Fout = dy.shape
    Fin = x.shape[1]
    assert tuple(dW.shape) == (Fout, Fin) and dW.stride(1) == 1
    if rows == 0:
        if not accumulate:
            dW.zero_()
            if db is not None:
                db.zero_()
        return
    nb = lib().gcl_linear_bwd_ws_bytes(rows, Fin, Fout)
    ws = workspace(nb, dy.device)
    _check(lib().gcl_dense_bwd_dw(_p(dy), _ld(dy), _p(x), _ld(x), int(act), _p(slope), _p(dW), dW.stride(0), _p(db), rows,
                                  Fin, Fout, 1 if accumulate else 0, ws.data_ptr(), ws.numel(), _stream()))


ACC_DW, ACC_DB, ACC_COLSUM = 1, 2, 4


class _RedSeg(C.Structure):
    _fields_ = [("out", C.c_void_p), ("poff", C.c_int32), ("count", C.c_int32), ("pld", C.c_int32), ("cols", C.c_int32),
                ("ldo", C.c_int32), ("acc", C.c_int32)]


class ReduceJob(C.Structure):
    _fields_ = [("part", C.c_void_p), ("pstride", C.c_int64), ("seg", _RedSeg * 3), ("spart", C.c_void_p),
                ("sout", C.c_void_p), ("nparts", C.c_int32), ("ns", C.c_int32)]


class _Deferred:

    def __init__(self):
        self.active = False
        self.jobs, self.dests, self.pool, self.used = [], set(), [], 0
        self.keep = []

    def ws(self, nbytes, device):
        if self.used == len(self.pool):
            self.pool.append(None)
        cur = self.pool[self.used]
        if cur is None or cur.numel() < nbytes or cur.device != torch.device(device):
            if cur is not None:
                _ws_retired.append(cur)
            cur = torch.empty(int(nbytes), dtype=torch.uint8, device=device)
            self.pool[self.used] = cur
        self.used += 1
        return cur


_deferred = _Deferred()


def defer_begin():
    _deferred.active = True


def defer_flush(close: bool = True, drop: bool = False):
    d = _deferred
    try:
        if d.jobs and not drop:
            arr = (ReduceJob * len(d.jobs))(*d.jobs)
            _check(lib().gcl_reduce_jobs(C.cast(arr, C.c_void_p), len(d.jobs), _stream()))
    finally:
        d.jobs, d.dests, d.used, d.keep = [], set(), 0, []
        if close:
            d.active = False


def linear_bwd_all(dy, W, x, in_slope, d_in_slope, dW, db, colsum_dx, acc_dW: bool, acc_db=None, acc_colsum=None,
                   act=None):
    acc_db = acc_dW if acc_db is None else acc_db
    acc_colsum = acc_dW if acc_colsum is None else acc_colsum
    a = _act_of(act, in_slope)
    if a == ACT_SILU:
        if db is not None and bool(acc_db) != bool(acc_dW):
            dense_bwd_dw(dy, x, dW, None, acc_dW, a, None)
            colsum(dy, db, acc_db)
        else:
            dense_bwd_dw(dy, x, dW, db, acc_dW, a, None)
        dx = dense_bwd_dx(dy, W, x, a, None, None)
        if colsum_dx is not None:
            colsum(dx, colsum_dx, acc_colsum)
        return dx
    rows, Fout = dy.shape
    Fin = W.shape[1]
    dx = torch.empty(rows, Fin, dtype=torch.float32, device=dy.device)
    nb = lib().gcl_linear_bwd_all_ws_bytes(rows, Fin, Fout)
    acc = (ACC_DW if acc_dW else 0) | (ACC_DB if acc_db else 0) | (ACC_COLSUM if acc_colsum else 0)
    d = _deferred
    if d.active:
        dests = {t.data_ptr() for t in (dW, db, colsum_dx) if t is not None}
        if dests & d.dests:
            defer_flush(close=False)
        ws = d.ws(nb, dy.device)
        job = ReduceJob()
        _check(lib().gcl_linear_bwd_all_deferred(
            _p(dy), _ld(dy), _p(W), _p(x), _ld(x), _p(in_slope), _p(d_in_slope), _p(dx), Fin, _p(dW), _p(db),
            _p(colsum_dx), rows, Fin, Fout, acc, ws.data_ptr(), ws.numel(), _stream(), C.byref(job)))
        if job.nparts > 0:
            d.jobs.append(job)
            d.dests |= dests
            d.keep.append((dW, db, colsum_dx, d_in_slope, ws))
        else:
            d.used -= 1
        return dx
    ws = workspace(nb, dy.device)
    _check(lib().gcl_linear_bwd_all(
        _p(dy), _ld(dy), _p(W), _p(x), _ld(x), _p(in_slope), _p(d_in_slope), _p(dx), Fin, _p(dW), _p(db),
        _p(colsum_dx), rows, Fin, Fout, acc, ws.data_ptr(), ws.numel(), _stream()))
    return dx


def aggregate(graph: Graph, h3, bias, transpose=False, out=None):
    B, n, F = h3.shape
    assert n == graph.n, f"graph has {graph.n} nodes, features have {n} rows"
    assert h3.stride(2) == 1
    if out is None:
        out = torch.empty(B, n, F, dtype=torch.float32, device=h3.device)
    tok = _probe_begin("aggregate", graph=graph, transpose=bool(transpose), B=B, F=F)
    _check(lib().gcl_aggregate(graph.handle, 1 if transpose else 0, _p(h3), h3.stride(1), h3.stride(0), _p(bias),
                               _p(out), out.stride(1), out.stride(0), B, F, _stream()))
    _probe_end(tok)
    return out


def layernorm_fwd(x, gamma, beta, eps=1e-5):
    rows, F = x.shape
    y = torch.empty(rows, F, dtype=torch.float32, device=x.device)
    stats = torch.empty(rows, 2, dtype=torch.float32, device=x.device)
    _check(lib().gcl_layernorm_fwd(_p(x), _ld(x), _p(gamma), _p(beta), float(eps), _p(y), F, _p(stats), rows, F, _stream()))
    return y, stats


def layernorm_fwd_map(x, gamma, beta, eps, out3, pos):
    rows, F = x.shape
    n_per = pos.numel()
    assert out3.stride(2) == 1 and rows % n_per == 0 and out3.shape[0] == rows // n_per
    stats = torch.empty(rows, 2, dtype=torch.float32, device=x.device)
    _check(lib().gcl_layernorm_fwd_map(_p(x), _ld(x), _p(gamma), _p(beta), float(eps), _p(out3), out3.stride(1), out3.stride(0),
                                       _pi(pos), n_per, _p(stats), rows, F, _stream()))
    return stats


def layernorm_bwd(dy, x, gamma, stats, dgamma, dbeta, accumulate: bool, colsum_dx=None, acc_colsum: bool = False,
                  dy_map=None):
    rows, F = x.shape
    dx = torch.empty(rows, F, dtype=torch.float32, device=x.device)
    nb = lib().gcl_layernorm_bwd_ws_bytes(rows, F)
    ws = workspace(nb, x.device)
    acc = (ACC_DW if accumulate else 0) | (ACC_COLSUM if acc_colsum else 0)
    if dy_map is not None:
        src3, pos = dy_map
        assert src3.stride(2) == 1 and src3.shape[2] >= F and rows % pos.numel() == 0 and src3.shape[0] == rows // pos.numel()
        _check(lib().gcl_layernorm_bwd_map(_p(src3), src3.stride(1), src3.stride(0), _pi(pos), pos.numel(), _p(x), _ld(x),
                                           _p(gamma), _p(stats), _p(dx), F, _p(dgamma), _p(dbeta), _p(colsum_dx), acc, rows, F,
                                           ws.data_ptr(), ws.numel(), _stream()))
        return dx
    _check(lib().gcl_layernorm_bwd_cs(_p(dy), _ld(dy), _p(x), _ld(x), _p(gamma), _p(stats), _p(dx), F, _p(dgamma),
                                      _p(dbeta), _p(colsum_dx), acc, rows, F, ws.data_ptr(), ws.numel(), _stream()))
    return dx


def graphnorm_fwd(x3, gamma, beta, eps=1e-5):
    B, n, F = x3.shape
    y = torch.empty(B, n, F, dtype=torch.float32, device=x3.device)
    stats = torch.empty(B, 2, dtype=torch.float32, device=x3.device)
    nb = lib().gcl_graphnorm_ws_bytes(B, n, F)
    ws = workspace(nb, x3.device)
    _check(lib().gcl_graphnorm_fwd(_p(x3), x3.stride(1), x3.stride(0), _p(gamma), _p(beta), float(eps), _p(y), F, n * F,
                                   _p(stats), B, n, F, ws.data_ptr(), ws.numel(), _stream()))
    return y, stats


def graphnorm_bwd(dy3, x3, gamma, stats, dgamma, dbeta, accumulate: bool, eps=1e-5):
    B, n, F = x3.shape
    dx = torch.empty(B, n, F, dtype=torch.float32, device=x3.device)
    nb = lib().gcl_graphnorm_ws_bytes(B, n, F)
    ws = workspace(nb, x3.device)
    _check(lib().gcl_graphnorm_bwd(_p(dy3), dy3.stride(1), dy3.stride(0), _p(x3), x3.stride(1), x3.stride(0), _p(gamma),
                                   _p(stats), float(eps), _p(dx), F, n * F, _p(dgamma), _p(dbeta),
                                   1 if accumulate else 0, B, n, F, ws.data_ptr(), ws.numel(), _stream()))
    return dx


def colsum(x, out, accumulate: bool):
    rows, F = x.shape
    nb = lib().gcl_colsum_ws_bytes(rows, F)
    ws = workspace(nb, x.device)
    _check(lib().gcl_colsum(_p(x), _ld(x), rows, F, _p(out), 1 if accumulate else 0, ws.data_ptr(), ws.numel(), _stream()))
    return out


def gat_tab_ok(graph: Graph, H: int, Cc: int) -> bool:
    return bool(lib().gcl_gat_tab_ok(graph.handle, H * Cc, int(H), int(Cc)))


def gat_fwd(graph: Graph, h3, att_src, att_dst, bias, H, Cc, need_alpha=True, tab=None):
    B, n, HC = h3.shape
    if tab is not None:
        n = graph.n
        assert h3.is_contiguous()
    dev = h3.device
    a_s = torch.empty(B, n, H, dtype=torch.float32, device=dev)
    a_d = torch.empty(B, n, H, dtype=torch.float32, device=dev)
    alpha = torch.empty(B, graph.e, H, dtype=torch.float32, device=dev) if need_alpha else None
    y = torch.empty(B, n, Cc, dtype=torch.float32, device=dev)
    tok = _probe_begin("gat_fwd", graph=graph, B=B, H=H, C=Cc, alpha=need_alpha)
    if tab is not None:
        _check(lib().gcl_gat_fwd_tab(graph.handle, _p(h3), h3.stride(1), h3.stride(0), _pi(tab), _p(att_src), _p(att_dst),
                                     _p(bias), _p(a_s), _p(a_d), _p(alpha), _p(y), Cc, n * Cc, B, H, Cc, _stream()))
    else:
        _check(lib().gcl_gat_fwd(graph.handle, _p(h3), h3.stride(1), h3.stride(0), _p(att_src), _p(att_dst), _p(bias),
                                 _p(a_s), _p(a_d), _p(alpha), _p(y), Cc, n * Cc, B, H, Cc, _stream()))
    _probe_end(tok)
    return y, a_s, a_d, alpha


def gat_bwd(graph: Graph, dy3, h3, att_src, att_dst, a_s, a_d, alpha, d_att_src, d_att_dst, d_bias, accumulate, H, Cc, tab=None):
    B, n, HC = h3.shape
    if tab is not None:
        n = graph.n
    dy3 = dy3.contiguous()
    dh = torch.empty(B, n, HC, dtype=torch.float32, device=h3.device)
    nb = lib().gcl_gat_bwd_ws_bytes(graph.e, n, B, H, Cc)
    ws = workspace(nb, h3.device)
    tok = _probe_begin("gat_bwd", graph=graph, B=B, H=H, C=Cc)
    if tab is not None:
        _check(lib().gcl_gat_bwd_tab(graph.handle, _p(dy3), Cc, n * Cc, _p(h3), h3.stride(1), h3.stride(0), _pi(tab), _p(att_src),
                                     _p(att_dst), _p(a_s), _p(a_d), _p(alpha), _p(dh), HC, n * HC, _p(d_att_src),
                                     _p(d_att_dst), _p(d_bias), 1 if accumulate else 0, B, H, Cc, ws.data_ptr(), ws.numel(),
                                     _stream()))
    else:
        _check(lib().gcl_gat_bwd(graph.handle, _p(dy3), Cc, n * Cc, _p(h3), h3.stride(1), h3.stride(0), _p(att_src),
                                 _p(att_dst), _p(a_s), _p(a_d), _p(alpha), _p(dh), HC, n * HC, _p(d_att_src), _p(d_att_dst),
                                 _p(d_bias), 1 if accumulate else 0, B, H, Cc, ws.data_ptr(), ws.numel(), _stream()))
    _probe_end(tok)
    return dh


def gat_alpha_edge_order(graph: Graph, alpha_slots_1sample, H):
    out = torch.empty(graph.e, H, dtype=torch.float32, device=alpha_slots_1sample.device)
    _check(lib().gcl_gat_alpha_to_edge_order(graph.handle, _p(alpha_slots_1sample.contiguous()), _p(out), H, _stream()))
    return out


def gat_prune(graph: Graph, alpha_edges, threshold: float) -> torch.Tensor:
    buf = torch.empty(2 * graph.e, dtype=torch.int64)
    kept = _i64(0)
    nb = lib().gcl_gat_prune_ws_bytes(graph.e)
    ws = workspace(nb, alpha_edges.device)
    _check(lib().gcl_gat_prune(graph.handle, _p(alpha_edges.contiguous()), float(threshold), buf.data_ptr(),
                               C.byref(kept), ws.data_ptr(), ws.numel(), _stream()))
    k = kept.value
    return buf[: 2 * k].view(2, k).clone()


def assemble_input(x3, grid_static, mesh_static, tail3=None):
    B, G, Cdyn = x3.shape
    M, Cs = mesh_static.shape
    x3 = x3.contiguous()
    out = torch.empty(B, G + M, Cdyn + Cs, dtype=torch.float32, device=x3.device)
    if tail3 is not None and tail3.is_contiguous() and tail3.shape[2] == Cdyn + Cs:
        _check(lib().gcl_assemble_input_tail(_p(x3), _p(grid_static), _p(mesh_static), _p(tail3), tail3.shape[1], _p(out),
                                             Cdyn + Cs, B, G, M, Cdyn, Cs, _stream()))
        return out
# ... 404 lines not shown
```

### graphcast-lite_amd/models.py

```python
import contextlib
import math
import os
import sys
from collections import OrderedDict
from typing import Optional, Tuple

import numpy as np
import torch
import torch.nn as nn

from . import hip
from .config import (
    DataConfig,
    GraphBlock,
    GraphBuildingConfig,
    GraphLayerType,
    MLPBlock,
    ModelConfig,
    PipelineConfig,
)
from .create_graphs import (create_decoding_graph, create_encoding_graph, create_processing_graph,
                            create_product_graph)
from .functional import (AssembleFn, EdgeLayout, GATLayerFn, Gather2Fn, GCNStackFn, GradLanding, GraphNormFn, InteractionNetFn,
                         LatSource, LayerNormFn, MeanAggFn, MeshLatFn, MLPFn)
# ... 495 lines not shown
            return False
        def ok(m):
            node_ln = all(ln.mode == "node" for ln in m.modules() if isinstance(ln, LayerNorm))
            return m.graph_layer.layer_type == GraphLayerType.ConvGCN and node_ln

        return ok(self.encoder) and ok(self.decoder) and getattr(self, "compact", True)

    _renumber_mesh = os.environ.get("GCL_NO_RENUMBER", "0") in ("0", "")

    def _mesh_order(self):
        if not self._renumber_mesh or self.processor.graph_layer.layer_type not in (
                GraphLayerType.ConvGCN, GraphLayerType.GATConv, GraphLayerType.SparseGATConv):
            return None
        cached = getattr(self, "_mesh_perm", None)
        if cached is None:
            M = self._num_mesh_nodes
            ei = self.processing_graph.detach().cpu()
            deg = torch.bincount(ei[1], minlength=M).numpy()
            order = torch.from_numpy(np.ascontiguousarray(tile_order(self._finest_mesh.vertices, 64, degree=deg))).to(torch.int64)
            pos = torch.empty(M, dtype=torch.int64)
            pos[order] = torch.arange(M)
            cached = self._mesh_perm = (order, pos)
        return cached

    def processor_graph(self) -> torch.Tensor:
        if self._compact_eligible() and self._mesh_order() is not None and not self.using_interaction_net:
            return self._processing_graph_tiled()
        return self.processing_graph

    def _processing_graph_tiled(self):
        g = self.processing_graph
        key = (id(g), g._version)
        c = getattr(self, "_proc_tiled", None)
        if c is None or c[0] != key:
            _, pos = self._mesh_order()
            c = self._proc_tiled = (key, pos.to(g.device)[g], g)
        return c[1]

    def _processing_graph_from_tiled(self, tiled: torch.Tensor) -> torch.Tensor:
        c = getattr(self, "_proc_tiled", None)
        if c is not None and c[1] is tiled:
            return c[2]
        order, _ = self._mesh_order()
        ref = order.to(tiled.device)[tiled]
        E = ref.shape[1]
        trail = (ref[0] == ref[1]).to(torch.int32).flip(0).cumprod(0).flip(0).bool()
        col = torch.arange(E, device=ref.device)
        key = torch.where(trail, (E - trail.sum()) + ref[0], col)
        ref = ref[:, torch.argsort(key, stable=True)]
        self._proc_tiled = ((id(ref), ref._version), tiled, ref)
        return ref

    def _compact_setup(self, device):
        G, M = self._num_grid_nodes, self._num_mesh_nodes
        enc, dec = self.encoding_graph.cpu(), self.decoding_graph.cpu()
        i32 = lambda t: t.to(torch.int32).contiguous().to(device)
        md = torch.unique(enc[1]) - G
        is_dep = torch.zeros(M, dtype=torch.bool)
        is_dep[md] = True
        mi = torch.nonzero(~is_dep).flatten()
        used = torch.unique(dec[0]) - G
        Md, Mi, U = md.numel(), mi.numel(), used.numel()
        remap_e = torch.full((G + M,), -1, dtype=torch.int64)
        remap_e[:G] = torch.arange(G)
        remap_e[G + md] = G + torch.arange(Md)
        remap_d = torch.full((G + M,), -1, dtype=torch.int64)
        remap_d[:G] = torch.arange(G)
        remap_d[G + used] = G + torch.arange(U)
        c = type("Compact", (), {})()
        c.Md, c.Mi, c.U = Md, Mi, U
        c.enc_graph = remap_e[enc].contiguous().to(device)
        c.dec_graph = remap_d[dec].contiguous().to(device)
        c.empty_graph = torch.zeros(2, 0, dtype=torch.int64, device=device)
        c.mstat_dep = self.init_mesh_features[md.to(self.init_mesh_features.device)].contiguous()
        Cdyn = self._dyn_size
        inv_stat = self.init_mesh_features[mi.to(self.init_mesh_features.device)]
        c.x_inv = torch.cat([torch.zeros(Mi, Cdyn, device=device), inv_stat.to(device)], dim=1).unsqueeze(0).contiguous()
        map_a = torch.full((M,), -1, dtype=torch.int64)
        map_a[md] = G + torch.arange(Md)
        map_b = torch.full((M,), -1, dtype=torch.int64)
        map_b[mi] = torch.arange(Mi)
        inv_a = torch.full((G + Md,), -1, dtype=torch.int64)
        inv_a[G:] = md
        perm = self._mesh_order()
        c.perm = perm
        if perm is not None:
            order, pos = perm
            map_a, map_b = map_a[order], map_b[order]
            inv_a[G:] = pos[md]
        c.maps_mesh = (i32(map_a), i32(map_b), i32(inv_a), i32(mi if perm is None else perm[1][mi]))
        dmap_a = torch.full((G + U,), -1, dtype=torch.int64)
        dmap_a[:G] = torch.arange(G)
        dmap_b = torch.full((G + U,), -1, dtype=torch.int64)
        dmap_b[G:] = used
        dinv_a = torch.full((G + Md,), -1, dtype=torch.int64)
        dinv_a[:G] = torch.arange(G)
        dinv_b = torch.full((M,), -1, dtype=torch.int64)
        dinv_b[used] = G + torch.arange(U)
        if perm is not None:
            dmap_b[G:] = perm[1][used]
            dinv_b = dinv_b[perm[0]]
        c.maps_dec = (i32(dmap_a), i32(dmap_b), i32(dinv_a), i32(dinv_b))
        c.fold = {}
        c.mi = mi
        self._compact = c
        return c

    _fold_invariant_rows = os.environ.get("GCL_NO_FOLD", "0") in ("0", "")

    def _fold_setup(self, c, B: int, device):
        G, M, Md, Mi = self._num_grid_nodes, self._num_mesh_nodes, c.Md, c.Mi
        r = -(-Mi // B)
        ne = G + Md + r
        Cs, Cdyn = self.init_mesh_features.shape[1], self._dyn_size
        f = type("Fold", (), {})()
        f.r, f.ne = r, ne
        stat = self.init_mesh_features.to(device)
        f.mstat = torch.cat([c.mstat_dep.to(device), torch.zeros(r, Cs, device=device)], dim=0).contiguous()
        x_fold = torch.zeros(B * r, Cdyn + Cs, device=device)
        x_fold[:Mi, Cdyn:] = stat[c.mi.to(device)]
        f.x_fold = x_fold.view(B, r, Cdyn + Cs)
        i32 = lambda t: t.to(torch.int32).contiguous().to(device)
        j = torch.arange(Mi)
        map_b = torch.full((M,), -1, dtype=torch.int64)
        map_b[c.mi] = (j // r) * ne + G + Md + (j % r)
        inv_fold = torch.full((B * r,), -1, dtype=torch.int64)
        inv_fold[:Mi] = c.mi
        if c.perm is not None:
            map_b = map_b[c.perm[0]]
            inv_fold[:Mi] = c.perm[1][c.mi]
        f.maps = (c.maps_mesh[0], i32(map_b), c.maps_mesh[2], i32(inv_fold))
        f.tab = torch.where(f.maps[0] >= 0, f.maps[0], -f.maps[1] - 1).to(torch.int32).contiguous()
        rd = -(-Md // B) if Md > 0 else 0
        f.rd, f.nm = rd, G + r + rd
        x_dep = torch.zeros(B * rd, Cdyn + Cs, device=device)
        x_dep[:Md, Cdyn:] = c.mstat_dep.to(device)
        f.x_tail2 = torch.cat([f.x_fold, x_dep.view(B, rd, Cdyn + Cs)], dim=1).contiguous()
        f.mstat2 = torch.zeros(r + rd, Cs, device=device)
        ea = torch.full((ne,), -1, dtype=torch.int64)
        ea[:G] = torch.arange(G)
        ea[G + Md:] = G + torch.arange(r)
        eb = torch.full((ne,), -1, dtype=torch.int64)
        d = torch.arange(Md)
        if rd > 0:
            eb[G: G + Md] = (d // rd) * f.nm + G + r + (d % rd)
        einv_a = torch.full((G + r,), -1, dtype=torch.int64)
        einv_a[:G] = torch.arange(G)
        einv_a[G:] = G + Md + torch.arange(r)
        einv_f = torch.full((B * rd,), -1, dtype=torch.int64)
        einv_f[:Md] = G + d
        f.maps_e = (i32(ea), i32(eb), i32(einv_a), i32(einv_f))
        dinv_a = torch.cat([c.maps_dec[2], torch.full((r,), -1, dtype=torch.int32, device=device)]).contiguous()
        f.maps_dec = (c.maps_dec[0], c.maps_dec[1], dinv_a, c.maps_dec[3])
        c.fold[B] = f
        return f

    def _forward_compact(self, X: torch.Tensor, attention_threshold=0.0, **kwargs):
        G, M = self._num_grid_nodes, self._num_mesh_nodes
        squeeze = X.dim() == 2 or (X.dim() == 3 and X.shape[0] == 1)
        X3 = X if X.dim() == 3 else X.unsqueeze(0)
        B = X3.shape[0]
        if self.use_product_graph:
            X3 = self._product_stage(X3)
        c = getattr(self, "_compact", None) or self._compact_setup(X3.device)
        if self._fold_invariant_rows:
            f = c.fold.get(B) or self._fold_setup(c, B, X3.device)
            if self._mlp_on_folded_rows and self.encoder.mlp is not None and f.rd > 0:
                x_m = AssembleFn.apply(X3, self.init_grid_features, f.mstat2, f.x_tail2)
                h_m = self.encoder.mlp(X=x_m)
                x_g = MeshLatFn.apply(h_m, f.maps_e, f.ne, G + f.r, f.rd, None)
                enc_c = self.encoder.graph_layer(X=x_g, edge_index=c.enc_graph)
            else:
                x_c = AssembleFn.apply(X3, self.init_grid_features, f.mstat, f.x_fold if f.r > 0 else None)
                enc_c = self.encoder.forward(X=x_c, edge_index=c.enc_graph)
            land = GradLanding(G) if kwargs.pop("_landing", False) and self._grad_landing else None
            lat_src = self._lat_source(c, f, enc_c, land)
            if lat_src is None:
                mesh_lat = MeshLatFn.apply(enc_c, f.maps, M, G + c.Md, f.r, land)
            maps_dec = f.maps_dec
        else:
            kwargs.pop("_landing", None)
            land = None
            lat_src = None
            maps_dec = c.maps_dec
            x_c = AssembleFn.apply(X3, self.init_grid_features, c.mstat_dep)
            enc_c = self.encoder.forward(X=x_c, edge_index=c.enc_graph)
            inv = self.encoder.forward(X=c.x_inv, edge_index=c.empty_graph) if c.Mi > 0 else None
            mesh_lat = Gather2Fn.apply(enc_c, inv, c.maps_mesh, M, B)
        if self.using_sparse_gat:
            pg = self._processing_graph_tiled() if c.perm is not None else self.processing_graph
            if land is not None and self._ln_into_decoder_input and self._latents_discarded and not squeeze:
                land.dec_buf = torch.empty(B, G + c.U, enc_c.shape[-1], dtype=torch.float32, device=enc_c.device)
                land.dec_map = maps_dec[3]
            processed, new_edge_index = self.processor.forward(
                X=mesh_lat, edge_index=pg, attention_threshold=attention_threshold,
                **({"_grad_src": land} if land is not None else {}), **kwargs)
            self.processing_graph = self._processing_graph_from_tiled(new_edge_index) if c.perm is not None else new_edge_index
        elif self.using_interaction_net:
            processed = self.processor.forward(X=mesh_lat, edge_index=self.processing_graph,
                                               attention_threshold=attention_threshold,
                                               edge_attr=self._processing_edge_features)
        else:
            pg = self._processing_graph_tiled() if c.perm is not None else self.processing_graph
            if (land is not None and self._ln_into_decoder_input and self._latents_discarded
                    and self.processor.graph_layer.layer_type in (GraphLayerType.ConvGCN, GraphLayerType.GATConv)
                    and not squeeze):
                land.dec_buf = torch.empty(B, G + c.U, enc_c.shape[-1], dtype=torch.float32, device=enc_c.device)
                land.dec_map = maps_dec[3]
            if lat_src is not None:
                processed = self.processor.forward(X=enc_c, edge_index=pg, attention_threshold=attention_threshold,
                                                   _lat_src=lat_src, **({"_grad_src": land} if land is not None else {}))
            else:
                processed = self.processor.forward(X=mesh_lat, edge_index=pg, attention_threshold=attention_threshold,
                                                   **({"_grad_src": land} if land is not None else {}))
        dec_in = Gather2Fn.apply(enc_c, processed, maps_dec, G + c.U, B, land)
        gcn_dec = self.decoder.graph_layer.layer_type == GraphLayerType.ConvGCN
        decoded = self.decoder.forward(X=dec_in, edge_index=c.dec_graph, **({"_out_rows": G} if gcn_dec else {}))
        out, grid_lat = (decoded if gcn_dec else decoded[:, :G, :]), enc_c[:, :G, :]
        if c.perm is not None and not self._want_prediction_only:
            pos_dev = getattr(c, "perm_pos_dev", None)
            if pos_dev is None or pos_dev.device != processed.device:
                pos_dev = c.perm_pos_dev = c.perm[1].to(processed.device)
            processed = processed.index_select(1, pos_dev)
        if squeeze:
            return out[0], grid_lat[0], processed[0]
        return out, grid_lat, processed

    _lat_through_table = os.environ.get("GCL_NO_LAT_TABLE", "0") in ("0", "")
    _mlp_on_folded_rows = os.environ.get("GCL_NO_MLP_FOLD", "0") in ("0", "")
    _ln_into_decoder_input = os.environ.get("GCL_NO_LN_MAP", "0") in ("0", "")
    _latents_discarded = False

    def _lat_source(self, c, f, enc_c, land):
        if not self._lat_through_table or c.perm is None or self.processor.mlp is not None:
            return None
        gl = self.processor.graph_layer
        if gl.layer_type == GraphLayerType.GATConv:
            first = gl.layers[0]
            if not isinstance(first, GATConv) or first.heads != 1 or enc_c.dim() != 3 or first.lin.weight.shape[1] != enc_c.shape[-1]:
                return None
            g = _graphs.get(self._processing_graph_tiled(), self._num_mesh_nodes, hip.GRAPH_GAT)
            if not hip.gat_tab_ok(g, 1, first.lin.weight.shape[0]):
                return None
            return LatSource(f.tab, f.maps, self._num_mesh_nodes, self._num_grid_nodes, c.Md, f.r, land)
        if gl.layer_type != GraphLayerType.ConvGCN:
            return None
        convs = [m for m in gl.layers if isinstance(m, GCNConv)]
        if not convs or enc_c.dim() != 3 or convs[0].lin.weight.shape[1] != enc_c.shape[-1]:
            return None
        g = _graphs.get(self._processing_graph_tiled(), self._num_mesh_nodes, hip.GRAPH_GCN)
        if not hip.gcn_layer_tab_ok(g, enc_c, convs[0].lin.weight.shape[0]):
            return None
        return LatSource(f.tab, f.maps, self._num_mesh_nodes, self._num_grid_nodes, c.Md, f.r, land)

    _want_prediction_only = False

    def forward_with_latents(self, X: torch.Tensor, attention_threshold=0.0, **kwargs):
        landing = kwargs.pop("_landing", False)
        self._want_prediction_only = landing
        if self._compact_eligible():
            return self._forward_compact(X, attention_threshold, _landing=landing, **kwargs)
        G = self._num_grid_nodes
        if X.dim() == 3 and X.shape[0] == 1:
            X = X.squeeze(0)
        if self.use_product_graph:
            X = self._product_stage(X)
        X = self._preprocess_input(grid_node_features=X)
        encoded = self.encoder.forward(X=X, edge_index=self.encoding_graph)
        grid_node_features = encoded[..., :G, :]
        mesh_node_features = encoded[..., G:, :]
        if self.using_sparse_gat:
            processed, new_edge_index = self.processor.forward(
                X=mesh_node_features, edge_index=self.processing_graph, attention_threshold=attention_threshold,
                **kwargs)
            self.processing_graph = new_edge_index
        elif self.using_interaction_net:
            processed = self.processor.forward(
                X=mesh_node_features, edge_index=self.processing_graph, attention_threshold=attention_threshold,
                edge_attr=self._processing_edge_features)
        else:
            processed = self.processor.forward(
                X=mesh_node_features, edge_index=self.processing_graph, attention_threshold=attention_threshold)
        processed_features = torch.cat((grid_node_features, processed), dim=-2)
        if self.decoder.graph_layer.layer_type == GraphLayerType.ConvGCN:
            decoded = self.decoder.forward(X=processed_features, edge_index=self.decoding_graph, _out_rows=G)
            return decoded, grid_node_features, processed
        decoded = self.decoder.forward(X=processed_features, edge_index=self.decoding_graph)
        return decoded[..., :G, :], grid_node_features, processed

    _grad_landing = os.environ.get("GCL_NO_LANDING", "0") in ("0", "")

    def forward(self, X: torch.Tensor, attention_threshold=0.0, **kwargs):
        self._latents_discarded = True
        try:
            return self.forward_with_latents(X, attention_threshold, _landing=True, **kwargs)[0]
        finally:
            self._latents_discarded = False
```

### include/gcl.h

```cpp
#ifndef GCL_H
#define GCL_H

#include <stddef.h>
#include <stdint.h>

#ifdef __cplusplus
extern "C" {
#endif

#define GCL_VERSION 100

#define GCL_OK 0
#define GCL_EINVAL (-1)
#define GCL_EHIP (-2)
#define GCL_ENOMEM (-3)
#define GCL_EUNSUPPORTED (-4)

typedef struct gcl_graph gcl_graph_t;
typedef void* gcl_stream_t;

int gcl_version(void);
const char* gcl_last_error(void);

#define GCL_GRAPH_GCN 0
#define GCL_GRAPH_GAT 1
#define GCL_GRAPH_MEAN 2

int gcl_graph_count_edges(const int64_t* edge_index, int64_t E, int32_t n, int32_t kind, int64_t* e_out);

int gcl_graph_build_host(const int64_t* edge_index, int64_t E, int32_t n, int32_t kind,
                         int32_t* rowptr, int32_t* col, float* w, int32_t* eperm,
                         int32_t* trowptr, int32_t* tcol, float* tw, int32_t* tslot);

int gcl_graph_create(const int64_t* edge_index, int64_t E, int32_t n, int32_t kind, gcl_graph_t** out);
void gcl_graph_destroy(gcl_graph_t* g);
int32_t gcl_graph_num_nodes(const gcl_graph_t* g);
int64_t gcl_graph_num_edges(const gcl_graph_t* g);
int32_t gcl_graph_max_in_degree(const gcl_graph_t* g);
int gcl_graph_export_edges(const gcl_graph_t* g, int64_t* edge_index_out);
const int32_t* gcl_graph_eperm_device(const gcl_graph_t* g);
int gcl_graph_halo_info(const gcl_graph_t* g, int32_t transpose, int32_t T, int32_t* out4);

int gcl_linear_fwd(const float* x, int64_t ldx, const float* in_slope, const float* W ,
                   const float* bias , float* y, int64_t ldy, int64_t rows,
                   int32_t Fin, int32_t Fout, gcl_stream_t stream);

int gcl_linear_bwd_dx(const float* dy, int64_t lddy, const float* W, const float* x, int64_t ldx,
                      const float* in_slope, float* d_in_slope, float* dx, int64_t lddx,
                      int64_t rows, int32_t Fin, int32_t Fout, void* ws, size_t ws_bytes,
                      gcl_stream_t stream);
int gcl_linear_bwd_dw(const float* dy, int64_t lddy, const float* x, int64_t ldx,
                      const float* in_slope, float* dW, float* db, int64_t rows, int32_t Fin,
                      int32_t Fout, int32_t accumulate, void* ws, size_t ws_bytes,
                      gcl_stream_t stream);
size_t gcl_linear_bwd_ws_bytes(int64_t rows, int32_t Fin, int32_t Fout);
#define GCL_ACC_DW 1
#define GCL_ACC_DB 2
#define GCL_ACC_COLSUM 4
int gcl_linear_bwd_all(const float* dy, int64_t lddy, const float* W, const float* x, int64_t ldx,
                       const float* in_slope, float* d_in_slope, float* dx, int64_t lddx, float* dW,
                       float* db, float* colsum_dx, int64_t rows, int32_t Fin, int32_t Fout,
                       int32_t accumulate, void* ws, size_t ws_bytes, gcl_stream_t stream);
size_t gcl_linear_bwd_all_ws_bytes(int64_t rows, int32_t Fin, int32_t Fout);

typedef struct gcl_reduce_job {
  const float* part;
  int64_t pstride;
  struct {
    float* out;
    int32_t poff, count, pld, cols, ldo, acc;
  } seg[3];
  const double* spart;
  float* sout;
  int32_t nparts, ns;
} gcl_reduce_job;
int gcl_linear_bwd_all_deferred(const float* dy, int64_t lddy, const float* W, const float* x, int64_t ldx,
                                const float* in_slope, float* d_in_slope, float* dx, int64_t lddx, float* dW,
                                float* db, float* colsum_dx, int64_t rows, int32_t Fin, int32_t Fout,
                                int32_t accumulate, void* ws, size_t ws_bytes, gcl_stream_t stream,
                                gcl_reduce_job* job);
int gcl_reduce_jobs(const gcl_reduce_job* jobs, int32_t n, gcl_stream_t stream);

#define GCL_ACT_NONE 0
#define GCL_ACT_PRELU 1
#define GCL_ACT_SILU 2
int gcl_dense_fwd(const float* x, int64_t ldx, int32_t act, const float* slope, const float* W,
                  int64_t ldw, const float* bias, const float* addend, int64_t ldadd, float* y,
                  int64_t ldy, int64_t rows, int32_t Fin, int32_t Fout, gcl_stream_t stream);
int gcl_dense_bwd_dx(const float* dy, int64_t lddy, const float* W, int64_t ldw, const float* z,
                     int64_t ldz, int32_t act, const float* slope, float* d_slope,
                     const float* addend, int64_t ldadd, float* dx, int64_t lddx, int64_t rows,
                     int32_t Fin, int32_t Fout, void* ws, size_t ws_bytes, gcl_stream_t stream);
int gcl_dense_bwd_dw(const float* dy, int64_t lddy, const float* x, int64_t ldx, int32_t act,
                     const float* slope, float* dW, int64_t lddw, float* db, int64_t rows,
                     int32_t Fin, int32_t Fout, int32_t accumulate, void* ws, size_t ws_bytes,
                     gcl_stream_t stream);

int gcl_aggregate(const gcl_graph_t* g, int32_t transpose, const float* h, int64_t ldh, int64_t bsh,
                  const float* bias, float* y, int64_t ldy, int64_t bsy, int32_t B, int32_t F,
                  gcl_stream_t stream);

int gcl_gat_fwd(const gcl_graph_t* g, const float* h, int64_t ldh, int64_t bsh,
                const float* att_src , const float* att_dst , const float* bias ,
                float* a_src , float* a_dst , float* alpha ,
                float* y, int64_t ldy, int64_t bsy, int32_t B, int32_t H, int32_t C,
                gcl_stream_t stream);
int gcl_gat_bwd(const gcl_graph_t* g, const float* dy, int64_t lddy, int64_t bsdy,
                const float* h, int64_t ldh, int64_t bsh, const float* att_src, const float* att_dst,
                const float* a_src, const float* a_dst, const float* alpha,
                float* dh, int64_t lddh, int64_t bsdh, float* d_att_src, float* d_att_dst,
                float* d_bias, int32_t accumulate, int32_t B, int32_t H, int32_t C,
                void* ws, size_t ws_bytes, gcl_stream_t stream);
size_t gcl_gat_bwd_ws_bytes(int64_t e_prime, int32_t n, int32_t B, int32_t H, int32_t C);
int gcl_gat_fwd_tab(const gcl_graph_t* g, const float* h, int64_t ldh, int64_t bsh, const int32_t* tab ,
                    const float* att_src, const float* att_dst, const float* bias, float* a_src, float* a_dst,
                    float* alpha, float* y, int64_t ldy, int64_t bsy, int32_t B, int32_t H, int32_t C,
                    gcl_stream_t stream);
int gcl_gat_bwd_tab(const gcl_graph_t* g, const float* dy, int64_t lddy, int64_t bsdy, const float* h, int64_t ldh,
                    int64_t bsh, const int32_t* tab , const float* att_src, const float* att_dst,
                    const float* a_src, const float* a_dst, const float* alpha, float* dh, int64_t lddh, int64_t bsdh,
                    float* d_att_src, float* d_att_dst, float* d_bias, int32_t accumulate, int32_t B, int32_t H,
                    int32_t C, void* ws, size_t ws_bytes, gcl_stream_t stream);
int gcl_gat_tab_ok(const gcl_graph_t* g, int64_t ldh, int32_t H, int32_t C);
int gcl_gat_alpha_to_edge_order(const gcl_graph_t* g, const float* alpha_slots, float* alpha_edges,
                                int32_t H, gcl_stream_t stream);
int gcl_gat_prune(const gcl_graph_t* g, const float* alpha_edges, float threshold,
                  int64_t* edge_index_out, int64_t* kept, void* ws, size_t ws_bytes,
                  gcl_stream_t stream);
size_t gcl_gat_prune_ws_bytes(int64_t e_prime);

int gcl_layernorm_fwd(const float* x, int64_t ldx, const float* gamma, const float* beta, float eps,
                      float* y, int64_t ldy, float* stats, int64_t rows, int32_t F,
                      gcl_stream_t stream);
int gcl_layernorm_fwd_map(const float* x, int64_t ldx, const float* gamma, const float* beta, float eps, float* y,
                          int64_t ldy, int64_t bsy, const int32_t* pos , int32_t n_per, float* stats,
                          int64_t rows, int32_t F, gcl_stream_t stream);
int gcl_layernorm_bwd(const float* dy, int64_t lddy, const float* x, int64_t ldx, const float* gamma,
                      const float* stats, float* dx, int64_t lddx, float* dgamma, float* dbeta,
                      int32_t accumulate, int64_t rows, int32_t F, void* ws, size_t ws_bytes,
                      gcl_stream_t stream);
int gcl_layernorm_bwd_cs(const float* dy, int64_t lddy, const float* x, int64_t ldx, const float* gamma,
                         const float* stats, float* dx, int64_t lddx, float* dgamma, float* dbeta,
                         float* colsum_dx, int32_t accumulate, int64_t rows, int32_t F, void* ws,
                         size_t ws_bytes, gcl_stream_t stream);
int gcl_layernorm_bwd_map(const float* dy, int64_t lddy, int64_t bsdy, const int32_t* pos, int32_t n_per,
                          const float* x, int64_t ldx, const float* gamma, const float* stats, float* dx,
                          int64_t lddx, float* dgamma, float* dbeta, float* colsum_dx, int32_t accumulate,
                          int64_t rows, int32_t F, void* ws, size_t ws_bytes, gcl_stream_t stream);
size_t gcl_layernorm_bwd_ws_bytes(int64_t rows, int32_t F);
int gcl_graphnorm_fwd(const float* x, int64_t ldx, int64_t bsx, const float* gamma, const float* beta,
                      float eps, float* y, int64_t ldy, int64_t bsy, float* stats, int32_t B,
                      int32_t n, int32_t F, void* ws, size_t ws_bytes, gcl_stream_t stream);
int gcl_graphnorm_bwd(const float* dy, int64_t lddy, int64_t bsdy, const float* x, int64_t ldx,
                      int64_t bsx, const float* gamma, const float* stats, float eps, float* dx,
                      int64_t lddx, int64_t bsdx, float* dgamma, float* dbeta, int32_t accumulate,
                      int32_t B, int32_t n, int32_t F, void* ws, size_t ws_bytes, gcl_stream_t stream);
size_t gcl_graphnorm_ws_bytes(int32_t B, int32_t n, int32_t F);

int gcl_colsum(const float* x, int64_t ldx, int64_t rows, int32_t F, float* out, int32_t accumulate,
               void* ws, size_t ws_bytes, gcl_stream_t stream);
size_t gcl_colsum_ws_bytes(int64_t rows, int32_t F);

int gcl_assemble_input(const float* x , const float* grid_static ,
                       const float* mesh_static , float* out, int64_t ldo, int32_t B,
                       int32_t G, int32_t M, int32_t Cdyn, int32_t Cs, gcl_stream_t stream);
int gcl_assemble_input_tail(const float* x, const float* grid_static, const float* mesh_static, const float* tail,
                            int32_t r, float* out, int64_t ldo, int32_t B, int32_t G, int32_t M, int32_t Cdyn,
                            int32_t Cs, gcl_stream_t stream);

int gcl_wmse_fwd_bwd(const float* delta, int64_t ldd, int64_t bsd, const float* x_last, int64_t ldx,
                     int64_t bsx, const float* y, int64_t ldy_, int64_t bsy, const float* node_w,
                     const float* chan_w, float inv_wsum, float grad_scale, float* d_delta,
                     float* out_state, const float* loss_prev, float* loss_out, int32_t B, int32_t G,
                     int32_t C, void* ws, size_t ws_bytes, gcl_stream_t stream);
size_t gcl_wmse_ws_bytes(int32_t B, int32_t G, int32_t C);

int gcl_adam_step(float* p, const float* g, float* m, float* v, int64_t count, float lr, float beta1,
                  float beta2, float eps, float weight_decay, int32_t step, float grad_scale,
                  gcl_stream_t stream);

int gcl_adam_step_dev(float* p, const float* g, float* m, float* v, int64_t count, float lr, float beta1,
                      float beta2, float eps, float weight_decay, int32_t* step_dev, float* bc_dev,
                      float grad_scale, gcl_stream_t stream);

int gcl_adam_step_groups(float* p, const float* g, float* m, float* v, int64_t count, const int32_t* chunk_param,
                         int32_t num_params, const int32_t* active, const float* lr, int32_t* step, float* bc,
                         float beta1, float beta2, float eps, float weight_decay, float grad_scale,
                         gcl_stream_t stream);

int gcl_copy_rows(const float* src, int64_t lds, int64_t bss, float* dst, int64_t ldd, int64_t bsd,
                  int32_t B, int32_t rows, int32_t F, gcl_stream_t stream);

int gcl_gcn_layer_fwd(const gcl_graph_t* g, const float* x, int64_t ldx, int64_t bsx, int32_t act,
                      const float* slope, const float* W , const float* bias, float* y,
                      int64_t ldy, int64_t bsy, int32_t B, int32_t Fin, int32_t Fout, int32_t Fout_store,
                      gcl_stream_t stream);
int gcl_gcn_layer_fwd_rows(const gcl_graph_t* g, const float* x, int64_t ldx, int64_t bsx, int32_t act,
                           const float* slope, const float* W , const float* bias, float* y,
                           int64_t ldy, int64_t bsy, int32_t B, int32_t Fin, int32_t Fout, int32_t Fout_store,
                           int32_t rows_out, gcl_stream_t stream);
int gcl_gcn_layer_fwd_tab(const gcl_graph_t* g, const float* x, int64_t ldx, int64_t bsx, int64_t x_rows,
                          const int32_t* tab , int32_t act, const float* slope, const float* W ,
                          const float* bias, float* y, int64_t ldy, int64_t bsy, int32_t B, int32_t Fin, int32_t Fout,
                          int32_t Fout_store, gcl_stream_t stream);
int gcl_gcn_layer_fwd_tab_ok(const gcl_graph_t* g, int64_t ldx, int64_t bsx, int64_t x_rows, int32_t B, int32_t Fin,
                             int32_t Fout);

int gcl_segment_reduce(const float* src, int64_t ld_src, int64_t bs_src, const int32_t* perm,
                       const int32_t* rowptr , int32_t mean, float* out, int64_t ld_out,
                       int64_t bs_out, int32_t B, int32_t n, int32_t D, gcl_stream_t stream);
int gcl_edge_combine(const float* base, const float* extra, const float* A, int64_t lda, int64_t bsa,
                     const int32_t* ia, const float* sa, const float* C, int64_t ldc, int64_t bsc,
                     const int32_t* ic, float* out, int32_t B, int64_t E, int32_t D,
                     gcl_stream_t stream);
int gcl_act_fwd(const float* x, float* y, int64_t count, int32_t act, const float* slope,
                gcl_stream_t stream);
int gcl_act_bwd(const float* x, const float* dy, float* dx, int64_t count, int32_t act,
                const float* slope, float* d_slope, void* ws, size_t ws_bytes, gcl_stream_t stream);
size_t gcl_act_bwd_ws_bytes(void);

int gcl_window_pack(const uint16_t* series , int64_t T, int32_t n_lon, int32_t n_lat,
                    int32_t Ct, const int64_t* t0, const float* mean, const float* stdv, int32_t C,
                    int32_t obs, int32_t pred, float* X , float* Y ,
                    int32_t B, gcl_stream_t stream);

int gcl_ar_advance(const float* state, const float* delta, int64_t ldd, int64_t bsd, const float* y_step,
                   int64_t ldy, int64_t bsy, const int32_t* chan_kind, float* new_state, float* out,
                   int64_t ldo, int64_t bso, int32_t out_off, int32_t B, int32_t G, int32_t obs, int32_t C,
                   int32_t residual, gcl_stream_t stream);
int gcl_ar_step_bwd(const float* dd, const float* g_loss, const float* g_new, const int32_t* chan_kind,
                    int32_t has_y, int32_t residual, float* d_delta, float* d_state, int32_t B, int32_t G,
                    int32_t obs, int32_t C, gcl_stream_t stream);

int gcl_pad_rows(const float* src, int64_t lds, int64_t bss, int32_t rows_src, int32_t F_src, float* dst,
// ... 82 lines not shown
```

Baseline: 25190.

## Add row-map addressing to x3 linear fwd/bwd kernels to avoid gather copies

Adds row-map variants of the x3 MFMA linear forward and fused backward kernels. These read and write rows through per-batch strides and an optional index table, so operands split across two buffers or permuted by a table are addressed in place. The model passes a latent dz table into LatSource so the processor path can use these kernels instead of materialising concatenated or gathered copies. This saves extra HBM traffic and launches, at the cost of index-table loads, more template instantiations and some register pressure.

Result: faster. 25550, median of 6 (+1.4%).

```diff
diff --git a/graphcast-lite_amd/csrc/linear.hip b/graphcast-lite_amd/csrc/linear.hip
--- a/graphcast-lite_amd/csrc/linear.hip
+++ b/graphcast-lite_amd/csrc/linear.hip
@@ -1208,6 +1208,22 @@
                                    Fout, nullptr, 0, nullptr, nullptr, nullptr, (hipStream_t)stream, act);
   return launch_gemm<EPI_BIAS>(x, ldx, act, act == GCL_ACT_PRELU ? slope : nullptr, W, ldw, 0, bias, y, ldy, rows, Fin,
                                Fout, nullptr, 0, addend, ldadd, nullptr, nullptr, (hipStream_t)stream);
+}
+
+extern "C" int gcl_dense_fwd_map_ok(const float* x, int64_t ldx, const gcl_row_map* mx, int32_t act, const float* y,
+                                    int64_t ldy, int64_t B, int64_t n, int32_t Fin, int32_t Fout) {
+  return !use_valu() && (act == GCL_ACT_NONE || act == GCL_ACT_PRELU) &&
+         gcl::x3_linear_fwd_map_applicable(x, ldx, mx, y, ldy, B, n, Fin, Fout, act);
+}
+
+extern "C" int gcl_dense_fwd_map(const float* x, int64_t ldx, const gcl_row_map* mx, int32_t act, const float* slope,
+                                 const float* W, const float* bias, float* y, int64_t ldy, int64_t B, int64_t n,
+                                 int32_t Fin, int32_t Fout, gcl_stream_t stream) {
+  GCL_CHECK_ARG(x && W && y, "dense_fwd_map: null argument");
+  if (int rc = check_act("dense_fwd_map", act, slope)) return rc;
+  if (!gcl_dense_fwd_map_ok(x, ldx, mx, act, y, ldy, B, n, Fin, Fout)) return GCL_EUNSUPPORTED;
+  return gcl::x3_linear_fwd_map(x, ldx, mx, act, act == GCL_ACT_PRELU ? slope : nullptr, W, bias, y, ldy, B, n, Fin,
+                                Fout, (hipStream_t)stream);
 }
 
 extern "C" int gcl_linear_fwd(const float* x, int64_t ldx, const float* in_slope, const float* W, const float* bias,
@@ -1393,16 +1409,26 @@
   return fused > sep ? fused : sep;
 }
 
+struct BwdMaps {
+  const gcl_row_map *dy, *x, *dx;
+  int64_t B, n;
+};
+
 static int bwd_all_impl(const float* dy, int64_t lddy, const float* W, const float* x, int64_t ldx,
                         const float* in_slope, float* d_in_slope, float* dx, int64_t lddx, float* dW,
                         float* db, float* colsum_dx, int64_t rows, int32_t Fin, int32_t Fout,
-                        int32_t accumulate, void* ws, size_t ws_bytes, gcl_stream_t stream, gcl_reduce_job* job) {
+                        int32_t accumulate, void* ws, size_t ws_bytes, gcl_stream_t stream, gcl_reduce_job* job,
+                        const BwdMaps* maps = nullptr) {
   if (job) memset(job, 0, sizeof(*job));
   GCL_CHECK_ARG(dy && W && x && dx && dW, "linear_bwd_all: null argument");
   GCL_CHECK_ARG(ws && ws_bytes >= gcl_linear_bwd_all_ws_bytes(rows, Fin, Fout), "linear_bwd_all: workspace too small");
   hipStream_t st = (hipStream_t)stream;
   const int acc_dw = (accumulate & GCL_ACC_DW) ? 1 : 0, acc_db = (accumulate & GCL_ACC_DB) ? 1 : 0,
             acc_cs = (accumulate & GCL_ACC_COLSUM) ? 1 : 0;
+  if (maps && !(fused_ok(dy, lddy, x, ldx, dx, lddx, Fin, Fout) && (Fin + 31) / 32 == 2 && !gcl::env_int("GCL_NO_FUSED64", 0) &&
+                gcl::x3_linear_bwd_map_applicable(dy, lddy, maps->dy, x, ldx, maps->x, dx, lddx, maps->dx, maps->B,
+                                                  maps->n, Fin, Fout)))
+    return GCL_EUNSUPPORTED;
   if (!fused_ok(dy, lddy, x, ldx, dx, lddx, Fin, Fout) || rows == 0) {
     int rc;
     if (db && acc_db != acc_dw) {
@@ -1433,7 +1459,12 @@
   float* part_cs = part_db + FoP;
   double* part_sl = (double*)(((uintptr_t)(part_dw + (size_t)3 * gcl::kNumCU * rec_f) + 15) & ~(uintptr_t)15);
   const bool want_slope = in_slope && d_in_slope;
-  if (use_x3) {
+  if (maps) {
+    if (int rc = gcl::x3_linear_bwd_map(dy, lddy, maps->dy, W, x, ldx, maps->x, in_slope, dx, lddx, maps->dx, maps->B,
+                                        maps->n, Fin, Fout, part_dw, db ? part_db : nullptr, colsum_dx ? part_cs : nullptr,
+                                        want_slope ? part_sl : nullptr, st))
+      return rc;
+  } else if (use_x3) {
     if (int rc = gcl::x3_linear_bwd(dy, lddy, W, x, ldx, in_slope, dx, lddx, rows, Fin, Fout, part_dw, db ? part_db : nullptr,
                                     colsum_dx ? part_cs : nullptr, want_slope ? part_sl : nullptr, st))
       return rc;
@@ -1518,6 +1549,37 @@
                       accumulate, ws, ws_bytes, stream, job);
 }
 
+extern "C" int gcl_linear_bwd_all_map_ok(const float* dy, int64_t lddy, const gcl_row_map* mdy, const float* x,
+                                         int64_t ldx, const gcl_row_map* mx, const float* dx, int64_t lddx,
+                                         const gcl_row_map* mdx, int64_t B, int64_t n, int32_t Fin, int32_t Fout) {
+  return fused_ok(dy, lddy, x, ldx, dx, lddx, Fin, Fout) && (Fin + 31) / 32 == 2 && !gcl::env_int("GCL_NO_FUSED64", 0) &&
+         gcl::x3_linear_bwd_map_applicable(dy, lddy, mdy, x, ldx, mx, dx, lddx, mdx, B, n, Fin, Fout);
+}
+
+extern "C" int gcl_linear_bwd_all_map(const float* dy, int64_t lddy, const gcl_row_map* mdy, const float* W,
+                                      const float* x, int64_t ldx, const gcl_row_map* mx, const float* in_slope,
+                                      float* d_in_slope, float* dx, int64_t lddx, const gcl_row_map* mdx, float* dW,
+                                      float* db, float* colsum_dx, int64_t B, int64_t n, int32_t Fin, int32_t Fout,
+                                      int32_t accumulate, void* ws, size_t ws_bytes, gcl_stream_t stream) {
+  GCL_CHECK_ARG(B >= 1 && n >= 1, "linear_bwd_all_map: bad shape B=%lld n=%lld", (long long)B, (long long)n);
+  const BwdMaps maps{mdy, mx, mdx, B, n};
+  return bwd_all_impl(dy, lddy, W, x, ldx, in_slope, d_in_slope, dx, lddx, dW, db, colsum_dx, B * n, Fin, Fout,
+                      accumulate, ws, ws_bytes, stream, nullptr, &maps);
+}
+
+extern "C" int gcl_linear_bwd_all_map_deferred(const float* dy, int64_t lddy, const gcl_row_map* mdy, const float* W,
+                                               const float* x, int64_t ldx, const gcl_row_map* mx,
+                                               const float* in_slope, float* d_in_slope, float* dx, int64_t lddx,
+                                               const gcl_row_map* mdx, float* dW, float* db, float* colsum_dx,
+                                               int64_t B, int64_t n, int32_t Fin, int32_t Fout, int32_t accumulate,
+                                               void* ws, size_t ws_bytes, gcl_stream_t stream, gcl_reduce_job* job) {
+  GCL_CHECK_ARG(job, "linear_bwd_all_map_deferred: null job");
+  GCL_CHECK_ARG(B >= 1 && n >= 1, "linear_bwd_all_map: bad shape B=%lld n=%lld", (long long)B, (long long)n);
+  const BwdMaps maps{mdy, mx, mdx, B, n};
+  return bwd_all_impl(dy, lddy, W, x, ldx, in_slope, d_in_slope, dx, lddx, dW, db, colsum_dx, B * n, Fin, Fout,
+                      accumulate, ws, ws_bytes, stream, job, &maps);
+}
+
 extern "C" int gcl_reduce_jobs(const gcl_reduce_job* jobs, int32_t n, gcl_stream_t stream) {
   GCL_CHECK_ARG(n >= 0 && (jobs || n == 0), "reduce_jobs: null argument");
   hipStream_t st = (hipStream_t)stream;
diff --git a/graphcast-lite_amd/csrc/linear_x3.hip b/graphcast-lite_amd/csrc/linear_x3.hip
--- a/graphcast-lite_amd/csrc/linear_x3.hip
+++ b/graphcast-lite_amd/csrc/linear_x3.hip
@@ -1,3 +1,5 @@
+#include <type_traits>
+
 #include "mfma_io.h"
 #include "x3.h"
 
@@ -19,6 +21,47 @@
 }
 using namespace gcl::mfma_io;
 using namespace gcl::x3;
+
+constexpr int kMap = 1, kTabY = 2, kTabP = 4, kTabX = 8;
+struct OpMap {
+  const unsigned char* a;
+  const unsigned char* b;
+  const int32_t* tab;
+  uint32_t bsa, bsb;
+  uint32_t lim_a, lim_b;
+};
+struct RowMaps {
+  OpMap y, p, x;
+  uint32_t n, m, s;
+};
+struct NoMaps {};
+template <int MAPS>
+using MapsArg = typename std::conditional<MAPS != 0, RowMaps, NoMaps>::type;
+
+struct RowPos {
+  uint32_t b, i;
+};
+__device__ __forceinline__ void split_row0(const RowMaps& mp, uint32_t u0, uint32_t& b0, uint32_t& i0) {
+  b0 = __umulhi(u0, mp.m) >> mp.s;
+  i0 = u0 - b0 * mp.n;
+}
+__device__ __forceinline__ RowPos row_pos(const RowMaps& mp, uint32_t b0, uint32_t i0, uint32_t k) {
+  const bool wr = i0 + k >= mp.n;
+  return RowPos{b0 + (wr ? 1u : 0u), i0 + k - (wr ? mp.n : 0u)};
+}
+__device__ __forceinline__ uint32_t map_off(const OpMap& m, uint32_t b, uint32_t i, uint32_t ldB) {
+  return b * m.bsa + i * ldB;
+}
+template <bool TAB>
+__device__ __forceinline__ const unsigned char* map_ptr(const OpMap& m, RowPos r, int32_t e, uint32_t ldB) {
+  if constexpr (!TAB) {
+    return m.a + map_off(m, r.b, r.i, ldB);
+  } else {
+    const bool in_a = e >= 0;
+    const uint32_t ri = in_a ? (uint32_t)e : ~(uint32_t)e;
+    return (in_a ? m.a : m.b) + ((in_a ? r.b * m.bsa : r.b * m.bsb) + ri * ldB);
+  }
+}
 
 constexpr int kRowB = 144;
 constexpr int kImgB = 32 * kRowB;
@@ -39,13 +82,14 @@
 #define X3_STAMP(slot) do {} while (0)
 #endif
 
-template <int NS, bool SILU, int NKS>
+template <int NS, bool SILU, int NKS, int MAPS>
 __global__ __launch_bounds__(256, 2) void linear_x3_fwd_kernel(const float* __restrict__ X, int64_t ldx,
                                                                const float* __restrict__ slope_p, int32_t akind,
                                                                const float* __restrict__ W,
                                                                const float* __restrict__ bias, float* __restrict__ Y,
                                                                int64_t ldy, int64_t rows, int32_t K, int32_t N,
-                                                               int32_t abl) {
+                                                               int32_t abl, const MapsArg<MAPS> mp) {
+  constexpr bool TP = (MAPS & kTabP) != 0;
   extern __shared__ __align__(16) unsigned char smem8[];
 #ifdef GCL_STAMPS
   const unsigned long long stamp_t0 = __builtin_amdgcn_s_memtime();
@@ -102,13 +146,27 @@
   const int rsub = lane >> 4, csub = lane & 15;
   const bool cok = csub * 4 < K;
   float4 pre[8];
+  int32_t tp[8];
   auto issue = [&](int64_t tile) {
     const int64_t r0 = tile * 128 + wave * 32;
-#pragma unroll
-    for (int it = 0; it < 8; ++it) {
-      const int64_t row = r0 + it * 4 + rsub;
-      const float4* p = (cok && row < rows_ld) ? reinterpret_cast<const float4*>(X + row * ldx + csub * 4) : zero4;
-      pre[it] = ld_stream(p);
+    if constexpr (MAPS != 0) {
+      uint32_t b0, i0, b1, i1;
+      split_row0(mp, (uint32_t)r0, b0, i0);
+      split_row0(mp, (uint32_t)(r0 + (int64_t)gridDim.x * 128), b1, i1);
+#pragma unroll
+      for (int it = 0; it < 8; ++it) {
+        const uint32_t k = it * 4 + rsub;
+        const unsigned char* px = map_ptr<TP>(mp.p, row_pos(mp, b0, i0, k), tp[it], (uint32_t)ldx * 4) + csub * 16;
+        pre[it] = ld_stream((cok && r0 + k < rows_ld) ? reinterpret_cast<const float4*>(px) : zero4);
+        if constexpr (TP) tp[it] = __builtin_nontemporal_load(mp.p.tab + row_pos(mp, b1, i1, k).i);
+      }
+    } else {
+#pragma unroll
+      for (int it = 0; it < 8; ++it) {
+        const int64_t row = r0 + it * 4 + rsub;
+        const float4* p = (cok && row < rows_ld) ? reinterpret_cast<const float4*>(X + row * ldx + csub * 4) : zero4;
+        pre[it] = ld_stream(p);
+      }
     }
   };
   auto commit = [&]() {
@@ -131,6 +189,12 @@
   };
 
   const int64_t ntiles = (rows + 127) / 128;
+  if constexpr (TP) {
+    uint32_t b0, i0;
+    split_row0(mp, (uint32_t)(blockIdx.x * 128 + wave * 32), b0, i0);
+#pragma unroll
+    for (int it = 0; it < 8; ++it) tp[it] = mp.p.tab[row_pos(mp, b0, i0, it * 4 + rsub).i];
+  }
   issue(blockIdx.x);
 #ifdef GCL_STAMPS
   unsigned long long stamp_acc[8] = {0, 0, 0, 0, 0, 0, 0, 0}, stamp_last = __builtin_amdgcn_s_memtime();
@@ -223,12 +287,13 @@
   return __builtin_shufflevector(a, b, 0, 1, 2, 3, 4, 5, 6, 7);
 }
 
-template <int NO>
+template <int NO, int MAPS>
 __global__ __launch_bounds__(256, 2) void linear_x3_bwd_kernel(
     const float* __restrict__ dY, int64_t lddy, const float* __restrict__ W, const float* __restrict__ P,
     int64_t ldp, const float* __restrict__ in_slope, float* __restrict__ dX, int64_t lddx, int64_t rows, int32_t Fin,
     int32_t Fout, float* __restrict__ part_dw, float* __restrict__ part_db, float* __restrict__ part_cs,
-    double* __restrict__ part_slope) {
+    double* __restrict__ part_slope, const MapsArg<MAPS> mp) {
+  constexpr bool TY = (MAPS & kTabY) != 0, TP = (MAPS & kTabP) != 0, TX = (MAPS & kTabX) != 0;
   constexpr int FoP = NO * 32, FiP = 64, NKO = NO * 2, NT = NO * 2;
   extern __shared__ __align__(16) unsigned char smem8[];
   unsigned char* Yimg = smem8;
@@ -278,14 +343,34 @@
   const unsigned ym0 = csub * 4 < Fout ? ~0u : 0u, ym1 = csub * 4 + 1 < Fout ? ~0u : 0u, ym2 = csub * 4 + 2 < Fout ? ~0u : 0u,
                  ym3 = csub * 4 + 3 < Fout ? ~0u : 0u;
   float4 pre_y[4], pre_p[4];
+  int32_t ty[4], tp[4], tx[4];
   auto issue = [&](int64_t tile) {
     const int64_t r0 = tile * 64 + wave * 16;
-#pragma unroll
-    for (int it = 0; it < 4; ++it) {
-      const int64_t row = r0 + it * 4 + rsub;
-      const bool rok = row < rows;
-      pre_y[it] = ld_stream((yok && rok) ? reinterpret_cast<const float4*>(dY + row * lddy + csub * 4) : zero4);
-      pre_p[it] = ld_stream((pok && rok) ? reinterpret_cast<const float4*>(P + row * ldp + csub * 4) : zero4);
+    if constexpr (MAPS != 0) {
+      uint32_t b0, i0, b1, i1;
+      split_row0(mp, (uint32_t)r0, b0, i0);
+      split_row0(mp, (uint32_t)(r0 + (int64_t)gridDim.x * 64), b1, i1);
+#pragma unroll
+      for (int it = 0; it < 4; ++it) {
+        const uint32_t k = it * 4 + rsub;
+        const bool rok = r0 + k < rows;
+        const RowPos rp = row_pos(mp, b0, i0, k);
+        const unsigned char* py = map_ptr<TY>(mp.y, rp, ty[it], (uint32_t)lddy * 4) + csub * 16;
+        const unsigned char* pp = map_ptr<TP>(mp.p, rp, tp[it], (uint32_t)ldp * 4) + csub * 16;
+        pre_y[it] = ld_stream((yok && rok) ? reinterpret_cast<const float4*>(py) : zero4);
+        pre_p[it] = ld_stream((pok && rok) ? reinterpret_cast<const float4*>(pp) : zero4);
+        const uint32_t inext = row_pos(mp, b1, i1, k).i;
+        if constexpr (TY) ty[it] = __builtin_nontemporal_load(mp.y.tab + inext);
+        if constexpr (TP) tp[it] = __builtin_nontemporal_load(mp.p.tab + inext);
+      }
+    } else {
+#pragma unroll
+      for (int it = 0; it < 4; ++it) {
+        const int64_t row = r0 + it * 4 + rsub;
+        const bool rok = row < rows;
+        pre_y[it] = ld_stream((yok && rok) ? reinterpret_cast<const float4*>(dY + row * lddy + csub * 4) : zero4);
+        pre_p[it] = ld_stream((pok && rok) ? reinterpret_cast<const float4*>(P + row * ldp + csub * 4) : zero4);
+      }
     }
   };
 
@@ -308,6 +393,18 @@
   double slope_acc = 0.0;
   float4 cur_p[4];
 
+  if constexpr (MAPS != 0) {
+    if constexpr (TY || TP) {
+      uint32_t b0, i0;
+      split_row0(mp, (uint32_t)(blockIdx.x * 64 + wave * 16), b0, i0);
+#pragma unroll
+      for (int it = 0; it < 4; ++it) {
+        const uint32_t i = row_pos(mp, b0, i0, it * 4 + rsub).i;
+        if constexpr (TY) ty[it] = mp.y.tab[i];
+        if constexpr (TP) tp[it] = mp.p.tab[i];
+      }
+    }
+  }
   issue(blockIdx.x);
 #ifdef GCL_STAMPS
   unsigned long long stamp_acc[8] = {0, 0, 0, 0, 0, 0, 0, 0}, stamp_last = __builtin_amdgcn_s_memtime();
@@ -317,6 +414,12 @@
     asm volatile("s_waitcnt vmcnt(0)" ::: "memory");
 #endif
     X3_STAMP(0);
+    if constexpr (TX) {
+      uint32_t b0, i0;
+      split_row0(mp, (uint32_t)(t * 64 + wave * 16), b0, i0);
+#pragma unroll
+      for (int it = 0; it < 4; ++it) tx[it] = __builtin_nontemporal_load(mp.x.tab + row_pos(mp, b0, i0, it * 4 + rsub).i);
+    }
 #pragma unroll
     for (int it = 0; it < 4; ++it) {
       float4 y = pre_y[it];
@@ -390,7 +493,34 @@
     __syncthreads();
     X3_STAMP(6);
 
-    {
+    if constexpr (MAPS != 0) {
+      const __amdgpu_buffer_rsrc_t ra = make_rsrc(mp.x.a, mp.x.lim_a), rb = make_rsrc(mp.x.b, TX ? mp.x.lim_b : 0);
+      const int64_t r0 = t * 64 + wave * 16;
+      uint32_t b0, i0;
+      split_row0(mp, (uint32_t)r0, b0, i0);
+#pragma unroll
+      for (int it = 0; it < 4; ++it) {
+        const int row = wave * 16 + it * 4 + rsub;
+        float4 v = *reinterpret_cast<const float4*>(Stg + row * 64 + csub * 4);
+        const float4 z = cur_p[it];
+        const bool nx = act && z.x <= 0.f, ny = act && z.y <= 0.f, nz = act && z.z <= 0.f, nw = act && z.w <= 0.f;
+        slope_acc += (double)(((nx ? v.x * z.x : 0.f) + (ny ? v.y * z.y : 0.f)) + ((nz ? v.z * z.z : 0.f) + (nw ? v.w * z.w : 0.f)));
+        v.x = nx ? v.x * slope : v.x; v.y = ny ? v.y * slope : v.y; v.z = nz ? v.z * slope : v.z; v.w = nw ? v.w * slope : v.w;
+        cs4.x += v.x; cs4.y += v.y; cs4.z += v.z; cs4.w += v.w;
+        const uint32_t k = it * 4 + rsub;
+        const bool ok = pok && r0 + k < rows;
+        const RowPos rp = row_pos(mp, b0, i0, k);
+        const uint32_t ldxB = (uint32_t)lddx * 4;
+        if constexpr (!TX) {
+          buf_st4<GCL_X3_ST_AUX>(ra, ok ? map_off(mp.x, rp.b, rp.i, ldxB) + csub * 16 : kOOB, v);
+        } else {
+          const int32_t e = tx[it];
+          const uint32_t ri = e >= 0 ? (uint32_t)e : ~(uint32_t)e;
+          buf_st4<GCL_X3_ST_AUX>(ra, (ok && e >= 0) ? rp.b * mp.x.bsa + ri * ldxB + csub * 16 : kOOB, v);
+          buf_st4<GCL_X3_ST_AUX>(rb, (ok && e < 0) ? rp.b * mp.x.bsb + ri * ldxB + csub * 16 : kOOB, v);
+        }
+      }
+    } else {
       const int64_t r0 = t * 64;
       const int64_t nr = (rows - r0) < 64 ? (rows - r0) : 64;
       const __amdgpu_buffer_rsrc_t rx = make_rsrc(dX + r0 * lddx, nr > 0 ? ((nr - 1) * lddx + Fin) * 4 : 0);
@@ -479,8 +609,8 @@
   const int grid = (int)(ntiles < 2 * kNumCU ? ntiles : 2 * kNumCU);
   const size_t lds = 4 * (size_t)kTileB;
 #define GCL_X3F3(NS_, SILU_, NKS_)                                                                                \
-  hipLaunchKernelGGL((linear_x3_fwd_kernel<NS_, SILU_, NKS_>), dim3(grid), dim3(256), lds, st, x, ldx, slope, akind, \
-                     W, bias, y, ldy, rows, K, N, x3_ablate())
+  hipLaunchKernelGGL((linear_x3_fwd_kernel<NS_, SILU_, NKS_, 0>), dim3(grid), dim3(256), lds, st, x, ldx, slope, akind, \
+                     W, bias, y, ldy, rows, K, N, x3_ablate(), NoMaps{})
 #define GCL_X3F(NS_, SILU_)           \
   do {                                \
     if (K <= 32) GCL_X3F3(NS_, SILU_, 2); \
@@ -520,10 +650,10 @@
   const size_t lds = 6 * (size_t)kImg64B + 64 * 64 * sizeof(float);
 #define GCL_X3B(NO_)                                                                                              \
   do {                                                                                                            \
-    auto kern = linear_x3_bwd_kernel<NO_>;                                                                        \
+    auto kern = linear_x3_bwd_kernel<NO_, 0>;                                                                     \
     GCL_ENSURE_DYN_LDS(kern, gcl::kLdsBytes);                                                                     \
     hipLaunchKernelGGL(kern, dim3(grid), dim3(256), lds, st, dy, lddy, W, x, ldx, in_slope, dx, lddx, rows, Fin, Fout, \
-                       part_dw, part_db, part_cs, part_slope);                                                    \
+                       part_dw, part_db, part_cs, part_slope, NoMaps{});                                          \
   } while (0)
   if (Fout > 32) GCL_X3B(2);
   else GCL_X3B(1);
@@ -533,3 +663,124 @@
 }
 
 }
+
+namespace {
+
+constexpr int64_t kMapLim = 0x7FFFFF00;
+
+bool make_op(OpMap& o, const float* a, const gcl_row_map* m, int64_t ld, int F, int64_t B, int64_t n) {
+  const gcl_row_map d = m ? *m : gcl_row_map{nullptr, nullptr, n * ld, 0, n, 0};
+  const float* b = (d.tab && d.b) ? d.b : a;
+  const int64_t bs_b = (d.tab && d.b) ? d.bs_b : d.bs_a, rows_b = (d.tab && d.b) ? d.rows_b : d.rows_a;
+  if (!a || !gcl::aligned16(a) || !gcl::aligned16(b) || (ld & 3) || ld < F || (d.bs_a & 3) || (bs_b & 3)) return false;
+  if (d.bs_a < 0 || bs_b < 0 || d.rows_a < 1 || rows_b < 1 || (!d.tab && d.rows_a < n)) return false;
+  const int64_t ext_a = ((B - 1) * d.bs_a + (d.rows_a - 1) * ld + F) * 4, ext_b = ((B - 1) * bs_b + (rows_b - 1) * ld + F) * 4;
+  if (ext_a >= kMapLim || ext_b >= kMapLim) return false;
+  o = OpMap{reinterpret_cast<const unsigned char*>(a), reinterpret_cast<const unsigned char*>(b), d.tab,
+            (uint32_t)(d.bs_a * 4), (uint32_t)(bs_b * 4), (uint32_t)ext_a, (uint32_t)ext_b};
+  return true;
+}
+
+bool make_div(RowMaps& mp, int64_t B, int64_t n) {
+  if (B < 1 || n < 32 || B * n + 2 * 2 * gcl::kNumCU * 128 >= ((int64_t)1 << 31)) return false;
+  int l = 0;
+  while (((int64_t)1 << l) < n) ++l;
+  const unsigned __int128 num = (unsigned __int128)1 << (31 + l);
+  mp.n = (uint32_t)n;
+  mp.m = (uint32_t)((num + n - 1) / n);
+  mp.s = (uint32_t)(l - 1);
+  return true;
+}
+
+}
+
+namespace gcl {
+
+bool x3_linear_fwd_map_applicable(const float* x, int64_t ldx, const gcl_row_map* mx, const float* y, int64_t ldy,
+                                  int64_t B, int64_t n, int K, int N, int akind) {
+  RowMaps mp{};
+  if (!x3_linear_fwd_applicable(x, ldx, y, ldy, K, N, akind) || akind == kActSilu) return false;
+  return make_div(mp, B, n) && make_op(mp.p, x, mx, ldx, K, B, n);
+}
+
+int x3_linear_fwd_map(const float* x, int64_t ldx, const gcl_row_map* mx, int akind, const float* slope, const float* W,
+                      const float* bias, float* y, int64_t ldy, int64_t B, int64_t n, int K, int N, hipStream_t st) {
+  RowMaps mp{};
+  if (!x3_linear_fwd_map_applicable(x, ldx, mx, y, ldy, B, n, K, N, akind) || !make_div(mp, B, n) ||
+      !make_op(mp.p, x, mx, ldx, K, B, n))
+    return GCL_EUNSUPPORTED;
+  const int64_t rows = B * n, ntiles = cdiv(rows, 128);
+  const int grid = (int)(ntiles < 2 * kNumCU ? ntiles : 2 * kNumCU);
+  const size_t lds = 4 * (size_t)kTileB;
+  const bool tab = mx && mx->tab;
+#define GCL_X3FM(NS_, NKS_)                                                                                          \
+  do {                                                                                                              \
+    if (tab)                                                                                                        \
+      hipLaunchKernelGGL((linear_x3_fwd_kernel<NS_, false, NKS_, kMap | kTabP>), dim3(grid), dim3(256), lds, st, x,  \
+                         ldx, slope, akind, W, bias, y, ldy, rows, K, N, 0, mp);                                    \
+    else                                                                                                            \
+      hipLaunchKernelGGL((linear_x3_fwd_kernel<NS_, false, NKS_, kMap>), dim3(grid), dim3(256), lds, st, x, ldx,    \
+                         slope, akind, W, bias, y, ldy, rows, K, N, 0, mp);                                         \
+  } while (0)
+  if (N > 32) {
+    if (K <= 32) GCL_X3FM(2, 2);
+    else GCL_X3FM(2, 4);
+  } else {
+    if (K <= 32) GCL_X3FM(1, 2);
+    else GCL_X3FM(1, 4);
+  }
+#undef GCL_X3FM
+  GCL_CHECK_LAUNCH();
+  return GCL_OK;
+}
+
+bool x3_linear_bwd_map_applicable(const float* dy, int64_t lddy, const gcl_row_map* mdy, const float* x, int64_t ldx,
+                                  const gcl_row_map* mx, const float* dx, int64_t lddx, const gcl_row_map* mdx,
+                                  int64_t B, int64_t n, int Fin, int Fout) {
+  RowMaps mp{};
+  if (!x3_linear_bwd_applicable(dy, lddy, x, ldx, dx, lddx, Fin, Fout)) return false;
+  if (mdy && mdy->tab && ((mx && mx->tab) || (mdx && mdx->tab))) return false;
+  return make_div(mp, B, n) && make_op(mp.y, dy, mdy, lddy, (Fout + 3) & ~3, B, n) && make_op(mp.p, x, mx, ldx, Fin, B, n) &&
+         make_op(mp.x, dx, mdx, lddx, Fin, B, n);
+}
+
+int x3_linear_bwd_map(const float* dy, int64_t lddy, const gcl_row_map* mdy, const float* W, const float* x,
+                      int64_t ldx, const gcl_row_map* mx, const float* in_slope, float* dx, int64_t lddx,
+                      const gcl_row_map* mdx, int64_t B, int64_t n, int Fin, int Fout, float* part_dw, float* part_db,
+                      float* part_cs, double* part_slope, hipStream_t st) {
+  RowMaps mp{};
+  if (!x3_linear_bwd_map_applicable(dy, lddy, mdy, x, ldx, mx, dx, lddx, mdx, B, n, Fin, Fout) || !make_div(mp, B, n) ||
+      !make_op(mp.y, dy, mdy, lddy, (Fout + 3) & ~3, B, n) || !make_op(mp.p, x, mx, ldx, Fin, B, n) ||
+      !make_op(mp.x, dx, mdx, lddx, Fin, B, n))
+    return GCL_EUNSUPPORTED;
+  const int64_t rows = B * n;
+  const int grid = x3_linear_bwd_blocks(rows);
+  const size_t lds = 6 * (size_t)kImg64B + 64 * 64 * sizeof(float);
+  const int tabs = (mdy && mdy->tab ? kTabY : 0) | (mx && mx->tab ? kTabP : 0) | (mdx && mdx->tab ? kTabX : 0);
+#define GCL_X3BM(NO_, T_)                                                                                          \
+  do {                                                                                                             \
+    auto kern = linear_x3_bwd_kernel<NO_, kMap | (T_)>;                                                            \
+    GCL_ENSURE_DYN_LDS(kern, gcl::kLdsBytes);                                                                      \
+    hipLaunchKernelGGL(kern, dim3(grid), dim3(256), lds, st, dy, lddy, W, x, ldx, in_slope, dx, lddx, rows, Fin, Fout, \
+                       part_dw, part_db, part_cs, part_slope, mp);                                                 \
+  } while (0)
+#define GCL_X3BT(NO_)                                    \
+  do {                                                   \
+    switch (tabs) {                                      \
+      case 0: GCL_X3BM(NO_, 0); break;                   \
+      case kTabY: GCL_X3BM(NO_, kTabY); break;           \
+      case kTabP: GCL_X3BM(NO_, kTabP); break;           \
+      case kTabX: GCL_X3BM(NO_, kTabX); break;           \
+      case kTabP | kTabX: GCL_X3BM(NO_, kTabP | kTabX); break; \
+      default: return GCL_EUNSUPPORTED;                  \
+    }                                                    \
+  } while (0)
+  if (Fout > 32) GCL_X3BT(2);
+  else GCL_X3BT(1);
+#undef GCL_X3BT
+#undef GCL_X3BM
+  GCL_CHECK_LAUNCH();
+  return GCL_OK;
+}
+
+}
diff --git a/graphcast-lite_amd/csrc/x3.h b/graphcast-lite_amd/csrc/x3.h
--- a/graphcast-lite_amd/csrc/x3.h
+++ b/graphcast-lite_amd/csrc/x3.h
@@ -13,6 +13,18 @@
 int x3_linear_bwd(const float* dy, int64_t lddy, const float* W, const float* x, int64_t ldx, const float* in_slope,
                   float* dx, int64_t lddx, int64_t rows, int Fin, int Fout, float* part_dw, float* part_db,
                   float* part_cs, double* part_slope, hipStream_t st);
+
+bool x3_linear_fwd_map_applicable(const float* x, int64_t ldx, const gcl_row_map* mx, const float* y, int64_t ldy,
+                                  int64_t B, int64_t n, int K, int N, int akind);
+int x3_linear_fwd_map(const float* x, int64_t ldx, const gcl_row_map* mx, int akind, const float* slope, const float* W,
+                      const float* bias, float* y, int64_t ldy, int64_t B, int64_t n, int K, int N, hipStream_t st);
+bool x3_linear_bwd_map_applicable(const float* dy, int64_t lddy, const gcl_row_map* mdy, const float* x, int64_t ldx,
+                                  const gcl_row_map* mx, const float* dx, int64_t lddx, const gcl_row_map* mdx,
+                                  int64_t B, int64_t n, int Fin, int Fout);
+int x3_linear_bwd_map(const float* dy, int64_t lddy, const gcl_row_map* mdy, const float* W, const float* x,
+                      int64_t ldx, const gcl_row_map* mx, const float* in_slope, float* dx, int64_t lddx,
+                      const gcl_row_map* mdx, int64_t B, int64_t n, int Fin, int Fout, float* part_dw, float* part_db,
+                      float* part_cs, double* part_slope, hipStream_t st);
 
 }
 
diff --git a/graphcast-lite_amd/functional.py b/graphcast-lite_amd/functional.py
--- a/graphcast-lite_amd/functional.py
+++ b/graphcast-lite_amd/functional.py
@@ -108,6 +108,12 @@
     nc = Md + r
     Fo = dz3.shape[-1]
     dz3 = dz3 if dz3.is_contiguous() else dz3.contiguous()
+    land = lat.landing
+    shared = land is not None and land.buf is not None
+    if want_dx and lat.dz_tab is not None:
+        dx = _lat_first_layer_bwd_mapped(lat, enc3, dz3, W, dW, acc_dw, Pc, (B, ne, D))
+        if dx is not False:
+            return dx
     dzc = torch.empty(B, nc, Fo, dtype=torch.float32, device=dz3.device)
     if Md > 0:
         hip.gather2_rows(dz3, inv_a[G: G + Md], None, None, Md, B, out=dzc[:, :Md])
@@ -118,8 +124,6 @@
         hip.copy_rows(tmp.view(B, r, Fo), dzc[:, Md:])
     if Pc is None:
         Pc = hip.copy_rows(enc3[:, G:, :], torch.empty(B, nc, D, dtype=torch.float32, device=dz3.device))
-    land = lat.landing
-    shared = land is not None and land.buf is not None
     if not want_dx:
         hip.linear_bwd_dw(dzc.view(B * nc, Fo), Pc.view(B * nc, D), None, dW, None, acc_dw)
         dxc = None
@@ -138,10 +142,36 @@
     return out
 
 
+def _lat_first_layer_bwd_mapped(lat, enc3, dz3, W, dW, acc_dw: bool, Pc, enc_shape):
+    _, _, inv_a, inv_fold = lat.maps
+    B, ne, D = enc_shape
+    G, Md, r = lat.G, lat.Md, lat.r
+    nc, Fo = Md + r, dz3.shape[-1]
+    land = lat.landing
+    shared = land is not None and land.buf is not None
+    out = land.buf if shared else torch.zeros(B, ne, D, dtype=torch.float32, device=dz3.device)
+    dzf = torch.empty(B, r, Fo, dtype=torch.float32, device=dz3.device) if r > 0 else None
+    dym = hip.row_map(dz3, lat.dz_tab, dzf)
+    xm = hip.row_map(Pc if Pc is not None else enc3[:, G:, :])
+    dxm = hip.row_map(out[:, G:])
+    if not hip.linear_bwd_all_map_ok(dym, xm, dxm, B, nc):
+        return False
+    if r > 1:
+        hip.gather2_rows(dz3, inv_fold, None, None, B * r, B, sum_batch=True, out=dzf, deal=r)
+    elif r == 1:
+        hip.copy_rows(hip.gather2_rows(dz3, inv_fold, None, None, B, B, sum_batch=True).view(B, 1, Fo), dzf)
+    hip.linear_bwd_all_map(dym, W, xm, dxm, B, nc, dW, acc_dW=acc_dw)
+    if shared:
+        land.buf, land.mesh_pending, land.handed_over = None, False, False
+        return None
+    return out
+
+
 class LatSource:
 
-    def __init__(self, tab, maps, M: int, G: int, Md: int, r: int, landing=None):
+    def __init__(self, tab, maps, M: int, G: int, Md: int, r: int, landing=None, dz_tab=None):
         self.tab, self.maps, self.M, self.G, self.Md, self.r, self.landing = tab, maps, M, G, Md, r, landing
+        self.dz_tab = dz_tab
         self._compact = {}
 
     def compact_tab(self, ne: int):
diff --git a/graphcast-lite_amd/hip.py b/graphcast-lite_amd/hip.py
--- a/graphcast-lite_amd/hip.py
+++ b/graphcast-lite_amd/hip.py
@@ -35,6 +35,13 @@
     "gcl_linear_bwd_all_deferred": (C.c_int, [_vp, _i64, _vp, _vp, _i64, _vp, _vp, _vp, _i64, _vp, _vp, _vp, _i64, _i32,
                                               _i32, _i32, _vp, _sz, _vp, _vp]),
     "gcl_reduce_jobs": (C.c_int, [_vp, _i32, _vp]),
+    "gcl_dense_fwd_map_ok": (C.c_int, [_vp, _i64, _vp, _i32, _vp, _i64, _i64, _i64, _i32, _i32]),
+    "gcl_dense_fwd_map": (C.c_int, [_vp, _i64, _vp, _i32, _vp, _vp, _vp, _vp, _i64, _i64, _i64, _i32, _i32, _vp]),
+    "gcl_linear_bwd_all_map_ok": (C.c_int, [_vp, _i64, _vp, _vp, _i64, _vp, _vp, _i64, _vp, _i64, _i64, _i32, _i32]),
+    "gcl_linear_bwd_all_map": (C.c_int, [_vp, _i64, _vp, _vp, _vp, _i64, _vp, _vp, _vp, _vp, _i64, _vp, _vp, _vp, _vp,
+                                         _i64, _i64, _i32, _i32, _i32, _vp, _sz, _vp]),
+    "gcl_linear_bwd_all_map_deferred": (C.c_int, [_vp, _i64, _vp, _vp, _vp, _i64, _vp, _vp, _vp, _vp, _i64, _vp, _vp, _vp,
+                                                  _vp, _i64, _i64, _i32, _i32, _i32, _vp, _sz, _vp, _vp]),
     "gcl_linear_bwd_all_ws_bytes": (_sz, [_i64, _i32, _i32]),
     "gcl_aggregate": (C.c_int, [_vp, _i32, _vp, _i64, _i64, _vp, _vp, _i64, _i64, _i32, _i32, _vp]),
     "gcl_gat_fwd": (C.c_int, [_vp, _vp, _i64, _i64, _vp, _vp, _vp, _vp, _vp, _vp, _vp, _i64, _i64, _i32, _i32, _i32, _vp]),
@@ -448,6 +455,72 @@
     return dx
 
 
+class RowMap(C.Structure):
+    _fields_ = [("b", C.c_void_p), ("tab", C.c_void_p), ("bs_a", C.c_int64), ("bs_b", C.c_int64),
+                ("rows_a", C.c_int64), ("rows_b", C.c_int64)]
+
+
+def row_map(a3, tab=None, b3=None):
+    if b3 is not None:
+        assert b3.stride(1) == a3.stride(1) and b3.stride(2) == 1
+    bs = lambda t: 0 if t.shape[0] == 1 else t.stride(0)
+    m = RowMap(_p(b3) if b3 is not None else None, _pi(tab) if tab is not None else None, bs(a3),
+               bs(b3) if b3 is not None else 0, a3.shape[1], b3.shape[1] if b3 is not None else 0)
+    return a3, m
+
+
+def dense_fwd_map_ok(xm, act, Fout: int, B: int, n: int) -> bool:
+    x3, m = xm
+    Fin = x3.shape[2]
+    probe = x3
+    return bool(lib().gcl_dense_fwd_map_ok(_p(x3), x3.stride(1), C.byref(m), int(act), _p(probe), Fout, B, n, Fin, Fout))
+
+
+def dense_fwd_map(xm, W, bias, B: int, n: int, act=ACT_NONE, slope=None):
+    x3, m = xm
+    Fout, Fin = W.shape
+    y = torch.empty(B * n, Fout, dtype=torch.float32, device=x3.device)
+    _check(lib().gcl_dense_fwd_map(_p(x3), x3.stride(1), C.byref(m), int(act), _p(slope), _p(W), _p(bias), _p(y), Fout,
+                                   B, n, Fin, Fout, _stream()))
+    return y
+
+
+def linear_bwd_all_map_ok(dym, xm, dxm, B: int, n: int) -> bool:
+    (dy3, mdy), (x3, mx), (dx3, mdx) = dym, xm, dxm
+    return bool(lib().gcl_linear_bwd_all_map_ok(_p(dy3), dy3.stride(1), C.byref(mdy), _p(x3), x3.stride(1), C.byref(mx),
+                                                 _p(dx3), dx3.stride(1), C.byref(mdx), B, n, x3.shape[2], dy3.shape[2]))
+
+
+def linear_bwd_all_map(dym, W, xm, dxm, B: int, n: int, dW, db=None, colsum_dx=None, acc_dW: bool = False,
+                       acc_db=None, acc_colsum=None, in_slope=None, d_in_slope=None):
+    (dy3, mdy), (x3, mx), (dx3, mdx) = dym, xm, dxm
+    acc_db = acc_dW if acc_db is None else acc_db
+    acc_colsum = acc_dW if acc_colsum is None else acc_colsum
+    Fout, Fin = dy3.shape[2], W.shape[1]
+    rows = B * n
+    nb = lib().gcl_linear_bwd_all_ws_bytes(rows, Fin, Fout)
+    acc = (ACC_DW if acc_dW else 0) | (ACC_DB if acc_db else 0) | (ACC_COLSUM if acc_colsum else 0)
+    args = (_p(dy3), dy3.stride(1), C.byref(mdy), _p(W), _p(x3), x3.stride(1), C.byref(mx), _p(in_slope), _p(d_in_slope),
+            _p(dx3), dx3.stride(1), C.byref(mdx), _p(dW), _p(db), _p(colsum_dx), B, n, Fin, Fout, acc)
+    d = _deferred
+    if d.active:
+        dests = {t.data_ptr() for t in (dW, db, colsum_dx) if t is not None}
+        if dests & d.dests:
+            defer_flush(close=False)
+        ws = d.ws(nb, dy3.device)
+        job = ReduceJob()
+        _check(lib().gcl_linear_bwd_all_map_deferred(*args, ws.data_ptr(), ws.numel(), _stream(), C.byref(job)))
+        if job.nparts > 0:
+            d.jobs.append(job)
+            d.dests |= dests
+            d.keep.append((dW, db, colsum_dx, d_in_slope, ws))
+        else:
+            d.used -= 1
+        return
+    ws = workspace(nb, dy3.device)
+    _check(lib().gcl_linear_bwd_all_map(*args, ws.data_ptr(), ws.numel(), _stream()))
+
+
 def aggregate(graph: Graph, h3, bias, transpose=False, out=None):
     B, n, F = h3.shape
     assert n == graph.n, f"graph has {graph.n} nodes, features have {n} rows"
diff --git a/graphcast-lite_amd/models.py b/graphcast-lite_amd/models.py
--- a/graphcast-lite_amd/models.py
+++ b/graphcast-lite_amd/models.py
@@ -671,6 +671,10 @@
         f.maps_e = (i32(ea), i32(eb), i32(einv_a), i32(einv_f))
         dinv_a = torch.cat([c.maps_dec[2], torch.full((r,), -1, dtype=torch.int32, device=device)]).contiguous()
         f.maps_dec = (c.maps_dec[0], c.maps_dec[1], dinv_a, c.maps_dec[3])
+        ia = c.maps_mesh[2][G: G + Md].to(torch.int64)
+        f.lat_dz_tab = None
+        if Md == 0 or bool((ia >= 0).all()):
+            f.lat_dz_tab = torch.cat([ia, -torch.arange(r, device=ia.device) - 1]).to(torch.int32).contiguous()
         c.fold[B] = f
         return f
 
@@ -748,6 +752,7 @@
     _lat_through_table = os.environ.get("GCL_NO_LAT_TABLE", "0") in ("0", "")
     _mlp_on_folded_rows = os.environ.get("GCL_NO_MLP_FOLD", "0") in ("0", "")
     _ln_into_decoder_input = os.environ.get("GCL_NO_LN_MAP", "0") in ("0", "")
+    _row_maps = os.environ.get("GCL_NO_ROW_MAPS", "0") in ("0", "")
     _latents_discarded = False
 
     def _lat_source(self, c, f, enc_c, land):
@@ -761,7 +766,8 @@
             g = _graphs.get(self._processing_graph_tiled(), self._num_mesh_nodes, hip.GRAPH_GAT)
             if not hip.gat_tab_ok(g, 1, first.lin.weight.shape[0]):
                 return None
-            return LatSource(f.tab, f.maps, self._num_mesh_nodes, self._num_grid_nodes, c.Md, f.r, land)
+            return LatSource(f.tab, f.maps, self._num_mesh_nodes, self._num_grid_nodes, c.Md, f.r, land,
+                             dz_tab=f.lat_dz_tab if self._row_maps else None)
         if gl.layer_type != GraphLayerType.ConvGCN:
             return None
         convs = [m for m in gl.layers if isinstance(m, GCNConv)]
@@ -770,7 +776,8 @@
         g = _graphs.get(self._processing_graph_tiled(), self._num_mesh_nodes, hip.GRAPH_GCN)
         if not hip.gcn_layer_tab_ok(g, enc_c, convs[0].lin.weight.shape[0]):
             return None
-        return LatSource(f.tab, f.maps, self._num_mesh_nodes, self._num_grid_nodes, c.Md, f.r, land)
+        return LatSource(f.tab, f.maps, self._num_mesh_nodes, self._num_grid_nodes, c.Md, f.r, land,
+                         dz_tab=f.lat_dz_tab if self._row_maps else None)
 
     _want_prediction_only = False
 
diff --git a/include/gcl.h b/include/gcl.h
--- a/include/gcl.h
+++ b/include/gcl.h
@@ -80,6 +80,32 @@
                                 int32_t accumulate, void* ws, size_t ws_bytes, gcl_stream_t stream,
                                 gcl_reduce_job* job);
 int gcl_reduce_jobs(const gcl_reduce_job* jobs, int32_t n, gcl_stream_t stream);
+
+typedef struct gcl_row_map {
+  const float* b;
+  const int32_t* tab;
+  int64_t bs_a, bs_b;
+  int64_t rows_a, rows_b;
+} gcl_row_map;
+int gcl_dense_fwd_map_ok(const float* x, int64_t ldx, const gcl_row_map* mx, int32_t act, const float* y, int64_t ldy,
+                         int64_t B, int64_t n, int32_t Fin, int32_t Fout);
+int gcl_dense_fwd_map(const float* x, int64_t ldx, const gcl_row_map* mx, int32_t act, const float* slope,
+                      const float* W, const float* bias, float* y, int64_t ldy, int64_t B, int64_t n, int32_t Fin,
+                      int32_t Fout, gcl_stream_t stream);
+int gcl_linear_bwd_all_map_ok(const float* dy, int64_t lddy, const gcl_row_map* mdy, const float* x, int64_t ldx,
+                              const gcl_row_map* mx, const float* dx, int64_t lddx, const gcl_row_map* mdx, int64_t B,
+                              int64_t n, int32_t Fin, int32_t Fout);
+int gcl_linear_bwd_all_map(const float* dy, int64_t lddy, const gcl_row_map* mdy, const float* W, const float* x,
+                           int64_t ldx, const gcl_row_map* mx, const float* in_slope, float* d_in_slope, float* dx,
+                           int64_t lddx, const gcl_row_map* mdx, float* dW, float* db, float* colsum_dx, int64_t B,
+                           int64_t n, int32_t Fin, int32_t Fout, int32_t accumulate, void* ws, size_t ws_bytes,
+                           gcl_stream_t stream);
+int gcl_linear_bwd_all_map_deferred(const float* dy, int64_t lddy, const gcl_row_map* mdy, const float* W,
+                                    const float* x, int64_t ldx, const gcl_row_map* mx, const float* in_slope,
+                                    float* d_in_slope, float* dx, int64_t lddx, const gcl_row_map* mdx, float* dW,
+                                    float* db, float* colsum_dx, int64_t B, int64_t n, int32_t Fin, int32_t Fout,
+                                    int32_t accumulate, void* ws, size_t ws_bytes, gcl_stream_t stream,
+                                    gcl_reduce_job* job);
 
 #define GCL_ACT_NONE 0
 #define GCL_ACT_PRELU 1
```
